# leonardsiegert/PULPo

Measured on AMD Instinct MI355X. Metric: volume-pairs/sec fwd+bwd, 160^3 fp32, higher is better.
Workload: dtype f32

## Files before the change

include/pulpo_hip.h:

```cpp
#ifndef PULPO_HIP_H
#define PULPO_HIP_H

#include <stddef.h>
#include <stdint.h>

#ifdef __cplusplus
extern "C" {
#endif

#define PULPO_ABI_VERSION 8
int pulpo_abi_version(void);
const char* pulpo_last_error(void);

size_t pulpo_conv3d_k3_packed_floats(int K, int N);
int pulpo_conv3d_k3_pack_weight(const float* w , float* wp, int Cin, int Cout, int dgrad, void* stream);
int pulpo_conv3d_k3_stat_tiles(int B, int D, int H, int W);
int pulpo_conv3d_k3_tile_config(int K, int N);
size_t pulpo_conv3d_k3_fwd_scratch_floats(int B, int D, int H, int W, int K, int N);
int pulpo_conv3d_k3_fwd(const float* in, int64_t in_bs, int64_t in_ps, int64_t in_cs, const float* wp, const float* bias, float* out,
                        int64_t out_bs, int64_t out_ps, int64_t out_cs, float* stats, float* scratch , int B,
                        int D, int H, int W, int K, int N, void* stream);
int pulpo_conv3d_k3_fwd_bn_lrelu(const float* in, int64_t in_bs, int64_t in_ps, int64_t in_cs, const float* wp, const float* bias,
                                 const float* coef, float slope, float* out, int64_t out_bs, int64_t out_ps, int64_t out_cs, float* scratch, int B,
                                 int D, int H, int W, int K, int N, void* stream);
int pulpo_conv3d_k3_algo(int B, int D, int H, int W, int K, int N);
size_t pulpo_conv3d_k3_packed_wino2_floats(int K, int N);
int pulpo_conv3d_k3_pack_weight_wino2(const float* w , float* wp, int Cin, int Cout, int dgrad, void* stream);
size_t pulpo_conv3d_k3_fwd_wino2_scratch_floats(int B, int D, int H, int W, int K, int N);
int pulpo_conv3d_k3_fwd_wino2(const float* in, int64_t in_bs, int64_t in_ps, int64_t in_cs, const float* wp, const float* bias, const float* coef,
                              float slope, float* out, int64_t out_bs, int64_t out_ps, int64_t out_cs, float* stats,
                              float* scratch , int B, int D, int H, int W, int K, int N, void* stream);
int pulpo_conv3d_k3_wino2_pipelined(int D, int H, int W, int K, int64_t in_ps);
int pulpo_conv3d_k3_dgrad_wino2_bnred_ok(int B, int D, int H, int W, int K, int N);
int pulpo_conv3d_k3_dgrad_wino2_bnred(const float* in, int64_t in_bs, int64_t in_ps, int64_t in_cs, const float* wp, float* out, int64_t out_bs,
                                      int64_t out_ps, const float* bn_y, int64_t bn_y_bs, int64_t bn_y_ps, const float* bn_coef, float slope,
                                      float* part, int B, int D, int H, int W, int K, int N, void* stream);
typedef struct PulpoPackJob {
    const float* w;
    float* wp;
    int Cin, Cout, dgrad, kind;
} PulpoPackJob;
int pulpo_conv3d_k3_pack_weights_multi(const PulpoPackJob* jobs, int njobs, void* stream);
size_t pulpo_conv3d_k3_wgrad_scratch_floats(int Cin, int Cout);
int pulpo_conv3d_k3_wgrad_algo(int B, int D, int H, int W, int Cin, int Cout, int vec);
int pulpo_conv3d_k3_wgrad(const float* in, int64_t in_bs, int64_t in_ps, int64_t in_cs, const float* dy, int64_t dy_bs, int64_t dy_ps,
                          int64_t dy_cs, float* dw, int accumulate, float* scratch, int B, int D, int H, int W, int Cin,
                          int Cout, void* stream);
typedef struct PulpoGradJob {
    const float* src;
    float* dst;
    int kind, a, b, c;
} PulpoGradJob;
int pulpo_grad_finish_multi(const PulpoGradJob* jobs, int njobs, void* stream);

size_t pulpo_conv3d_k3_packed_bf16_elems(int K, int N);
int pulpo_conv3d_k3_pack_weight_bf16(const float* w , uint16_t* wp, int Cin, int Cout, int dgrad, void* stream);
size_t pulpo_conv3d_k3_fwd_bf16_scratch_floats(int B, int D, int H, int W, int K, int N);
int pulpo_conv3d_k3_fwd_bf16_stat_tiles(int B, int D, int H, int W);
int pulpo_conv3d_k3_fwd_bf16(const float* in, int64_t in_bs, int64_t in_ps, int64_t in_cs, const uint16_t* wp, const float* bias, float* out,
                             int64_t out_bs, int64_t out_ps, int64_t out_cs, float* stats, float* scratch, int B, int D, int H, int W, int K,
                             int N, void* stream);
int pulpo_conv3d_k3_fwd_bn_lrelu_bf16(const float* in, int64_t in_bs, int64_t in_ps, int64_t in_cs, const uint16_t* wp, const float* bias,
                                      const float* coef, float slope, float* out, int64_t out_bs, int64_t out_ps, int64_t out_cs, float* scratch,
                                      int B, int D, int H, int W, int K, int N, void* stream);
int pulpo_conv3d_k3_wgrad_bf16(const float* in, int64_t in_bs, int64_t in_ps, int64_t in_cs, const float* dy, int64_t dy_bs, int64_t dy_ps,
                               int64_t dy_cs, float* dw, int accumulate, float* scratch , int B, int D,
                               int H, int W, int Cin, int Cout, void* stream);

int pulpo_colsum(const float* partials, int nrow, int ncol, float* out, float scale, int accumulate, void* stream);
size_t pulpo_bn_fwd_finalize_scratch_doubles(int ntile, int C);
int pulpo_bn_fwd_finalize(const float* stats, int ntile, int C, double count, const float* gamma, const float* beta, float* running_mean,
                          float* running_var, int64_t* num_batches_tracked , float momentum, float eps, float* coef,
                          double* scratch, void* stream);
int pulpo_bn_eval_coef(const float* gamma, const float* beta, const float* running_mean, const float* running_var, float eps, int C,
                       float* coef, void* stream);
int pulpo_bn_lrelu_apply(const float* y, int64_t yps, float* z, int64_t zps, const float* coef, int64_t npix, int C, float slope, void* stream);
int pulpo_bn_lrelu_apply_pool2_ok(int C, int64_t yps, int64_t zps, int64_t pps);
int pulpo_bn_lrelu_apply_pool2(const float* y, int64_t yps, float* z, int64_t zps, float* pooled, int64_t pps, const float* coef, int B, int D, int H,
                               int W, int C, float slope, void* stream);
int pulpo_bn_bwd_blocks(int64_t npix, int C);
int pulpo_avgpool2_bwd_bnred(const float* gout, int64_t gops, const float* add, int64_t aps, float* gin, int64_t gips, const float* y, int64_t yps,
                             const float* coef, float slope, float* partial, int B, int D, int H, int W, int C, void* stream);
int pulpo_bn_lrelu_bwd_reduce(const float* dz, int64_t dzps, const float* y, int64_t yps, const float* coef, int64_t npix, int C, float slope,
                              float* partial , void* stream);
size_t pulpo_bn_bwd_finalize_scratch_doubles(int nrow, int C);
int pulpo_bn_bwd_finalize(const float* rows, int nrow, int C, const float* coef, double count, int use_means, float* dbeta, float* dgamma,
                          int accumulate, double* totd , double* scratch, void* stream);
int pulpo_bn_lrelu_bwd_apply(const float* dz, int64_t dzps, const float* y, int64_t yps, const float* coef, const double* totd, float* dy,
                             int64_t dyps, int64_t npix, int C, float slope, float* partial2 , void* stream);

int pulpo_heads_fwd(const float* h, int64_t ps, const float* Wt, const float* bias, const float* eps, float* o0, float* o1, float* o2, int nout,
                    int B, int64_t V, int C, void* stream);
int pulpo_heads_bwd_blocks(int B, int64_t V, int C);
int pulpo_heads_bwd(const float* h, int64_t ps, const float* Wt, const float* g0, const float* g1, const float* g2, const float* eps,
                    const float* sigma, float* dh, int64_t dps, float* partial , int nout, int B, int64_t V, int C,
                    void* stream);

int pulpo_avgpool2_fwd(const float* in, int64_t ips, float* out, int64_t ops, int B, int D, int H, int W, int C, void* stream);
int pulpo_avgpool2_bwd(const float* gout, int64_t gops, float* gin, int64_t gips, int B, int D, int H, int W, int C, void* stream);
int pulpo_avgpool2_bwd_add(const float* gout, int64_t gops, const float* add, int64_t aps, float* gin, int64_t gips, int B, int D, int H, int W,
                           int C, void* stream);
int pulpo_resize_trilinear_fwd(const float* in, const float* add, float* out, int64_t nplanes, int Di, int Hi, int Wi, int Do, int Ho, int Wo,
                               float mult, void* stream);
int pulpo_resize_trilinear_bwd(const float* gout, float* gin, int64_t nplanes, int Di, int Hi, int Wi, int Do, int Ho, int Wo, float mult,
                               void* stream);
int pulpo_resize_trilinear_scaled_fwd(const float* in, const float* add, float* out, int64_t nplanes, int Di, int Hi, int Wi, int Do, int Ho,
                                      int Wo, float scale_d, float scale_h, float scale_w, float mult, void* stream);
int pulpo_resize_trilinear_scaled_bwd(const float* gout, float* gin, int64_t nplanes, int Di, int Hi, int Wi, int Do, int Ho, int Wo,
                                      float scale_d, float scale_h, float scale_w, float mult, void* stream);
int pulpo_feedback_up2_fwd(const float* const* srcs , const int* chans , int nsrc, float* out, int64_t ops,
                           int B, int Di, int Hi, int Wi, void* stream);
int pulpo_feedback_up2_bwd(const float* gout, int64_t gops, float* const* gsrcs , const int* chans, int nsrc,
                           int B, int Di, int Hi, int Wi, void* stream);

int pulpo_warp3d_fwd(const float* df, const float* img, float* out, int B, int C, int Dg, int Hg, int Wg, int Di, int Hi, int Wi, void* stream);
int pulpo_warp_mask_fwd(const float* df, const float* mask, float* out, int B, int Dg, int Hg, int Wg, int Di, int Hi, int Wi, void* stream);
int pulpo_warp3d_bwd(const float* df, const float* img, const float* gout, float* gdf, float* gimg, int B, int C, int Dg, int Hg, int Wg, int Di,
                     int Hi, int Wi, void* stream);
int pulpo_vecint_fwd(const float* v, float* work, int B, int D, int H, int W, int nsteps, void* stream);
size_t pulpo_vecint_bwd_tmp_floats(int B, int D, int H, int W, int nsteps);
int pulpo_vecint_bwd(const float* work, const float* gout, float* gin, float* tmp , int B, int D, int H, int W,
                     int nsteps, void* stream);

int pulpo_loss_blocks(int64_t n);
int pulpo_ncc_fwd(const float* I, const float* J, float* S , float* T , float* partial, int B, int D, int H, int W,
                  int win, void* stream);
int pulpo_ncc_bwd(const float* I, const float* J, const float* S, float* T , const float* gscale, float coef, float* gJ, int B, int D,
                  int H, int W, int win, void* stream);
int pulpo_ncc_masked_fwd(const float* I, const float* J, const float* wa, const float* wb , float* S ,
                         float* T , float* partial , int B, int D, int H, int W, int win, void* stream);
int pulpo_ncc_masked_bwd(const float* I, const float* J, const float* S, const float* wa, const float* wb , float* T ,
                         const float* gscale, float coef, float* gJ, int B, int D, int H, int W, int win, void* stream);
int pulpo_masked_finish(const float* partial, int nblk, double scale, int root, double count, float* out , void* stream);
int pulpo_mind_blocks(int B, int D, int H, int W, int d);
int pulpo_mind_descriptor(const float* I, float* out , int B, int D, int H, int W, int d, float eps, void* stream);
int pulpo_mind_fwd(const float* y_true, const float* y_pred, const float* wa , const float* wb , float* partial, int B, int D,
                   int H, int W, int d, float eps, void* stream);
int pulpo_mind_bwd(const float* y_true, const float* y_pred, const float* wa , const float* wb , float* scratch ,
                   const float* gscale, float coef, float* gpred, int B, int D, int H, int W, int d, float eps, void* stream);
int pulpo_mi_blocks(int B, int64_t V);
int64_t pulpo_mi_scratch_floats(int B, int64_t V, int K);
int pulpo_mi_fwd(const float* y_true, const float* y_pred, const float* wa , const float* wb , float* scratch, double* p,
                 double* mi, float* G, float* loss, int B, int64_t V, int K, double gamma, void* stream);
int pulpo_mi_bwd(const float* y_true, const float* y_pred, const float* wa , const float* wb , const float* G,
                 const float* gscale, float coef, float* gpred, int B, int64_t V, int K, void* stream);
int pulpo_kl_fwd(const float* mu, const float* sigma, const float* mu1 , const float* sigma1 , int64_t n,
                 float* partial, void* stream);
int pulpo_kl_bwd(const float* mu, const float* sigma, const float* mu1, const float* sigma1, const float* gscale, float coef, float* gmu,
                 float* gsigma, int64_t n, void* stream);
int pulpo_l2reg_fwd(const float* df, int64_t nplanes, int D, int H, int W, float* partial, void* stream);
int pulpo_l2reg_bwd(const float* df, const float* gscale, float coef, float* gdf, int64_t nplanes, int D, int H, int W, void* stream);
int pulpo_bending_blocks(int64_t nplanes, int D, int H, int W);
int pulpo_bending_fwd(const float* df, int64_t nplanes, int D, int H, int W, float* partial, void* stream);
int pulpo_bending_bwd(const float* df, const float* gscale, float coef, float* gdf, int64_t nplanes, int D, int H, int W, void* stream);
int pulpo_weighted_sum_fwd(const float* terms, const float* weights, int n, float scale, int scaled, float* levels, float* total, void* stream);
int pulpo_weighted_sum_bwd(const float* gtotal, const float* glevels, const float* weights, int n, float scale, float* gterms, void* stream);

int pulpo_metric_blocks(int64_t n);
int pulpo_sqdiff_fwd(const float* a, const float* b, int64_t n, float* partial, void* stream);
int pulpo_sqdiff_bwd(const float* a, const float* b, const float* gscale, float coef, float* ga, int64_t n, void* stream);
int pulpo_sqdiff_masked_fwd(const float* a, const float* b, const float* wa, const float* wb ,
                            float* partial , int B, int C, int64_t V, void* stream);
int pulpo_sqdiff_masked_bwd(const float* a, const float* b, const float* wa, const float* wb , const float* gscale, float coef, float* ga,
                            int B, int C, int64_t V, void* stream);
int pulpo_dice_blocks(int64_t V);
int pulpo_dice_fwd(const float* inp, const float* tgt, int nplanes, int64_t V, float dice_factor, float* partial, double* numden, float* loss,
                   void* stream);
int pulpo_dice_bwd(const float* inp, const float* tgt, const double* numden, const float* gscale, int nplanes, int64_t V, float dice_factor,
                   float* ginp, void* stream);
int pulpo_jacdet_fwd(const float* df, float* out, double* partial , int B, int D, int H, int W, int normalize, void* stream);
int pulpo_jdetstd_finalize(const double* partial, int64_t n, float lamb, double* stat, float* loss, void* stream);
int pulpo_kl_nondiag_fwd(const float* mu, const float* sigma, int64_t nplanes, int D, int H, int W, float prior_lambda, float* partial, float* loss,
                         void* stream);
int pulpo_kl_nondiag_bwd(const float* mu, const float* sigma, const float* gscale, int64_t nplanes, int D, int H, int W, float prior_lambda,
                         float* gmu, float* gsigma, void* stream);
int pulpo_jdetstd_bwd(const float* df, const float* jdet, const double* stat, const float* gscale, float lamb, float* gdf, int B, int D, int H, int W,
                      int normalize, void* stream);

int pulpo_rmse(const float* a, const float* b, int64_t n, float* partial , float* out, void* stream);
int pulpo_dsc(const float* inp, const float* tgt, int nplanes, int64_t V, float* partial , float* out,
              void* stream);
int pulpo_percent_leq0(const float* x, int64_t n, float* partial , float* out, void* stream);
int pulpo_warp_landmarks(const float* lm , const float* df , float* out , int nlm, int nsamp,
                         int nd, int D, int H, int W, int* flag, void* stream);
int pulpo_field_quality_blocks(int B, int D, int H, int W);
size_t pulpo_field_quality_ws_bytes(int B, int D, int H, int W);
int pulpo_field_quality(const float* df, float* out , void* ws, int B, int D, int H, int W, int normalize, void* stream);

size_t pulpo_vecint_pair_scratch_floats(int B, int D, int H, int W, int nsteps);
int pulpo_vecint_pair_fwd(const float* v, float* fwd, float* inv, float* scratch , int B, int D, int H, int W, int nsteps,
                          void* stream);
size_t pulpo_inverse_consistency_ws_bytes(int B, int D, int H, int W);
int pulpo_inverse_consistency(const float* a, const float* b, float* out , void* ws, int B, int D, int H, int W, void* stream);
int pulpo_transport_points(const float* pts , const float* field , float* out , int npts,
                           int nsamp, int nd, int D, int H, int W, int* flag, void* stream);

int pulpo_affine_field(const float* theta, float* out, int B, int D, int H, int W, void* stream);
int pulpo_affine_warp_fwd(const float* theta, const float* img, float* out, int B, int C, int Dg, int Hg, int Wg, int Di, int Hi, int Wi, void* stream);
size_t pulpo_affine_warp_bwd_ws_bytes(int B, int Dg, int Hg, int Wg);
int pulpo_affine_warp_bwd(const float* theta, const float* img, const float* gout, float* gtheta , void* ws, int B, int C, int Dg, int Hg,
                          int Wg, int Di, int Hi, int Wi, void* stream);
int pulpo_affine_compose(const float* theta, const float* df, float* out, int B, int Dg, int Hg, int Wg, int Di, int Hi, int Wi, void* stream);

int pulpo_mc_moments_update(const float* sample, float* mean, float* m2, int64_t n, int k, void* stream);
int pulpo_mc_moments_std(const float* m2, const float* scale , float* out , int B, int C, int64_t V, int k, void* stream);

size_t pulpo_warp_labels_ws_bytes(int B, int C);
int pulpo_warp_labels(const float* df, const void* labels, int ldt, int C, const void* target , float* onehot ,
                      void* amax , float* dice , float* mean , float* m2 ,
                      int k, void* ws, int* flag, int B, int Dg, int Hg, int Wg, int Di, int Hi, int Wi, void* stream);
int pulpo_labels_check(const void* labels, int ldt, int64_t n, int C, int* flag, void* stream);
int pulpo_warp_labels_soft_dice(const float* df, const void* labels, const void* target, int ldt, int C, float* dice, float* mean, void* ws,
                                int* flag, int B, int Dg, int Hg, int Wg, int Di, int Hi, int Wi, int Dt, int Ht, int Wt, void* stream);
int pulpo_labels_from_onehot(const float* seg, void* labels, int ldt, int B, int C, int64_t V, void* stream);
int pulpo_map_ncc_blocks(int64_t n);
int pulpo_map_ncc(const float* a, const float* b, int64_t n, double* partial, double* out, void* stream);
int pulpo_label_dice_fwd(const float* df, const void* labels, const void* target, int ldt, int C, float dice_factor, float* loss, float* dice,
                         float* coef, void* ws, int* flag, int B, int Dg, int Hg, int Wg, int Di, int Hi, int Wi, int Dt, int Ht, int Wt,
                         void* stream);
int pulpo_label_dice_bwd(const float* df, const void* labels, const void* target, int ldt, int C, const float* coef, const float* gup, float* ddf,
                         int B, int Dg, int Hg, int Wg, int Di, int Hi, int Wi, int Dt, int Ht, int Wt, void* stream);
int pulpo_labels_pool2(const void* labels, int ldt, int C, float* out, int B, int D, int H, int W, void* stream);
int pulpo_labels_resize(const void* labels, int ldt, int C, float* out, int B, int Dt, int Ht, int Wt, int Do, int Ho, int Wo, void* stream);

#define PULPO_EDT_INF (1 << 29)
int pulpo_edt_sq(const void* mask, int* out, int B, int D, int H, int W, void* stream);
int64_t pulpo_surface_distances_bins(int D, int H, int W);
size_t pulpo_surface_distances_ws_bytes(int B, int C, int D, int H, int W);
int pulpo_surface_distances(const void* lab_a, const void* lab_b, int ldt, int C, double q, float* out, int* hist , void* ws, int* flag,
                            int B, int D, int H, int W, int nd, void* stream);

int pulpo_augment_apply(const float* theta, const float* phi, int spacing, int Gz, int Gy, int Gx, const float* img, float* img_out, int C,
                        const float* mask, float* mask_out, int Cm, const void* labels, void* labels_out, int ldt, const float* iparams, int iflags,
                        const float* bias, int Lz, int Ly, int Lx, const void* seed, float fill, int fill_label, int B, int D, int H, int W,
                        void* stream);
int pulpo_bspline_field(const float* phi, const float* theta, float* out, int spacing, int Gz, int Gy, int Gx, int B, int D, int H, int W, void* stream);
int pulpo_philox4x32(const void* counters, const void* key, void* out, int64_t n, void* stream);

int pulpo_adam_step(float* p, const float* g, float* m, float* v, int64_t n, float lr, double beta1, double beta2, float eps, int step, float gscale,
                    void* stream);
int pulpo_anchored_adam_step(float* p, const float* g, float* m, float* v, const float* mean, const float* prec, int64_t n, float lr, double beta1,
                             double beta2, float eps, int step, float* partial, void* stream);

size_t pulpo_conv3d_k3_packed_wino3_floats(int K, int N);
int pulpo_conv3d_k3_pack_weight_wino3(const float* w , float* wp, int Cin, int Cout, int dgrad, void* stream);
int pulpo_conv3d_k3_fwd_wino3(const float* in, int64_t in_bs, int64_t in_ps, int64_t in_cs, const float* wp, const float* bias, const float* coef,
                              float slope, float* out, int64_t out_bs, int64_t out_ps, int64_t out_cs, float* stats, int B, int D, int H, int W, int K,
                              int N, void* stream);
int pulpo_conv3d_k3_dgrad_wino3_bnred(const float* in, int64_t in_bs, int64_t in_ps, int64_t in_cs, const float* wp, float* out, int64_t out_bs,
                                      int64_t out_ps, const float* bn_y, int64_t bn_y_bs, int64_t bn_y_ps, const float* bn_coef, float slope, float* part,
                                      int B, int D, int H, int W, int K, int N, void* stream);
int pulpo_conv3d_k3_wino3g_ok(int B, int D, int H, int W, int K, int N);
size_t pulpo_conv3d_k3_fwd_wino3g_scratch_floats(int B, int D, int H, int W, int K, int N);
int pulpo_conv3d_k3_fwd_wino3g(const float* in, int64_t in_bs, int64_t in_ps, int64_t in_cs, const float* wp, const float* bias, const float* coef,
                               float slope, float* out, int64_t out_bs, int64_t out_ps, int64_t out_cs, float* stats, float* scratch, int B, int D,
                               int H, int W, int K, int N, void* stream);

int pulpo_conv3d_k3_fwd_bf16_t(const void* in, int64_t in_bs, int64_t in_ps, int64_t in_cs, const uint16_t* wp, const float* bias, void* out,
                               int64_t out_bs, int64_t out_ps, int64_t out_cs, int dt, float* stats, float* scratch, int B, int D, int H, int W,
                               int K, int N, void* stream);
int pulpo_conv3d_k3_fwd_bn_lrelu_bf16_t(const void* in, int64_t in_bs, int64_t in_ps, int64_t in_cs, const uint16_t* wp, const float* bias,
                                        const float* coef, float slope, void* out, int64_t out_bs, int64_t out_ps, int64_t out_cs, int dt,
                                        float* scratch, int B, int D, int H, int W, int K, int N, void* stream);
int pulpo_conv3d_k3_wgrad_bf16_t(const void* in, int64_t in_bs, int64_t in_ps, int64_t in_cs, const void* dy, int64_t dy_bs, int64_t dy_ps,
                                 int64_t dy_cs, int dt, float* dw, int accumulate, float* scratch, int B, int D, int H, int W, int Cin, int Cout,
                                 void* stream);
int pulpo_conv3d_k3_fwd_bf16_kernel(int B, int D, int H, int W, int K, int N, int dt, int64_t in_ps, int64_t out_ps);
int pulpo_conv3d_k3_wgrad_bf16_kernel(int B, int D, int H, int W, int Cin, int Cout, int dt, int64_t in_ps, int64_t dy_ps);
int pulpo_bn_lrelu_apply_t(const void* y, int y_dt, int64_t yps, void* z, int z_dt, int64_t zps, const float* coef, int64_t npix, int C, float slope,
                           void* stream);
int pulpo_bn_lrelu_apply_pool2_t(const void* y, int y_dt, int64_t yps, void* z , int z_dt, int64_t zps,
                                 void* pooled , int64_t pps,
                                 const float* coef, int B, int D, int H, int W, int C, float slope, void* stream);
int pulpo_bn_lrelu_bwd_reduce_t(const void* dz, int dz_dt, int64_t dzps, const void* y, int y_dt, int64_t yps, const float* coef, int64_t npix, int C,
                                float slope, float* partial, void* stream);
int pulpo_bn_lrelu_bwd_apply_t(const void* dz, int dz_dt, int64_t dzps, const void* y, int y_dt, int64_t yps, const float* coef, const double* totd,
                               void* dy , int64_t dyps, int64_t npix, int C, float slope, float* partial2, void* stream);
int pulpo_avgpool2_bwd_bnred_t(const void* gout, int64_t gops, const void* add, int64_t aps, void* gin, int64_t gips, int g_dt ,
                               const void* y, int y_dt, int64_t yps, const float* coef, float slope, float* partial, int B, int D, int H, int W,
                               int C, void* stream);
int pulpo_heads_fwd_t(const void* h, int h_dt, int64_t ps, const float* Wt, const float* bias, const float* eps, float* o0, float* o1, float* o2,
                      int nout, int B, int64_t V, int C, void* stream);
int pulpo_heads_bwd_t(const void* h, int h_dt, int64_t ps, const float* Wt, const float* g0, const float* g1, const float* g2, const float* eps,
                      const float* sigma, void* dh , int64_t dps, float* partial, int nout, int B, int64_t V, int C, void* stream);
int pulpo_avgpool2_fwd_t(const void* in, int64_t ips, void* out, int64_t ops, int dt, int B, int D, int H, int W, int C, void* stream);
int pulpo_avgpool2_bwd_t(const void* gout, int64_t gops, const void* add , int64_t aps, void* gin, int64_t gips, int dt, int B, int D,
                         int H, int W, int C, void* stream);
int pulpo_feedback_up2_fwd_t(const float* const* srcs , const int* chans , int nsrc, void* out,
                             int dt, int64_t ops, int B, int Di, int Hi, int Wi, void* stream);
int pulpo_feedback_up2_bwd_t(const void* gout, int dt, int64_t gops, float* const* gsrcs , const int* chans,
                             int nsrc, int B, int Di, int Hi, int Wi, void* stream);

int pulpo_conv3d_k3_wgrad_bn_rows(int B, int D, int H, int W, int Cout);
int pulpo_conv3d_k3_wgrad_bn(const float* in, int64_t in_bs, int64_t in_ps, int64_t in_cs, const void* dz, int dz_dt, int64_t dz_bs, int64_t dz_ps,
                             const float* y, int64_t y_bs, int64_t y_ps, const float* coef, const double* totd, float slope, float* dw,
                             int accumulate, float* scratch, float* part2, int B, int D, int H, int W, int Cin, int Cout, void* stream);

int pulpo_bn_lrelu_bwd_apply_pooled_t(const void* gout, int64_t gops, const void* add , int64_t aps, int g_dt, const void* y, int y_dt,
                                      int64_t yps, const float* coef, const double* totd, void* dy , int64_t dyps, float slope,
                                      float* partial2, int B, int D, int H, int W, int C, void* stream);

int pulpo_bn_lrelu_apply_kb(const float* y, int64_t yps, float* z, int64_t zps, int64_t zkb, const float* coef, int64_t npix, int C, float slope, void* stream);
int pulpo_bn_lrelu_bwd_apply_kb_t(const void* dz, int dz_dt, int64_t dzps, int64_t dzkb, const float* y, int64_t yps, const float* coef, const double* totd,
                                  float* dy, int64_t dyps, int64_t dykb, int64_t npix, int C, float slope, float* partial2, void* stream);
int pulpo_conv3d_k3_wgrad_bn_kb(const float* in, int64_t in_bs, int64_t in_ps, int64_t in_cs, const float* dz, int64_t dz_bs, int64_t dz_ps, int64_t dz_kb,
                                const float* y, int64_t y_bs, int64_t y_ps, const float* coef, const double* totd, float slope, float* dw, int accumulate,
                                float* scratch, float* part2, int B, int D, int H, int W, int Cin, int Cout, void* stream);
int pulpo_bn_lrelu_bwd_apply_pooled_kb_t(const void* gout, int64_t gops, const void* add , int64_t aps, int g_dt, const float* y, int64_t yps,
                                         const float* coef, const double* totd, float* dy, int64_t dyps, int64_t dykb, float slope, float* partial2,
                                         int B, int D, int H, int W, int C, void* stream);
int pulpo_conv3d_k3_fwd_wino3_kb(const float* in, int64_t in_bs, int64_t in_ps, int64_t in_kb, const float* wp, const float* bias, const float* coef,
                                 float slope, float* out, int64_t out_bs, int64_t out_ps, int64_t out_kb, float* stats, int B, int D, int H, int W, int K,
                                 int N, void* stream);
int pulpo_conv3d_k3_dgrad_wino3_bnred_kb(const float* in, int64_t in_bs, int64_t in_ps, int64_t in_kb, const float* wp, float* out, int64_t out_bs,
                                         int64_t out_ps, int64_t out_kb, const float* bn_y, int64_t bn_y_bs, int64_t bn_y_ps, const float* bn_coef, float slope,
                                         float* part, int B, int D, int H, int W, int K, int N, void* stream);
int pulpo_conv3d_k3_wgrad_kb(const float* in, int64_t in_bs, int64_t in_ps, int64_t in_kb, const float* dy, int64_t dy_bs, int64_t dy_ps, int64_t dy_kb,
                             float* dw, int accumulate, float* scratch, float* slabs , int nslab, int B, int D, int H, int W, int Cin, int Cout,
                             void* stream);

int pulpo_conv3d_k3_wgrad_det_slabs(int Cin, int Cout);
int pulpo_conv3d_k3_wgrad_det(const float* in, int64_t in_bs, int64_t in_ps, int64_t in_cs, const float* dy, int64_t dy_bs, int64_t dy_ps,
                              int64_t dy_cs, float* dw, int accumulate, float* scratch, float* slabs, int nslab, int B, int D, int H, int W,
                              int Cin, int Cout, void* stream);
int pulpo_conv3d_k3_wgrad_bf16_det_t(const void* in, int64_t in_bs, int64_t in_ps, int64_t in_cs, const void* dy, int64_t dy_bs, int64_t dy_ps,
                                     int64_t dy_cs, int dt, float* dw, int accumulate, float* scratch, float* slabs, int nslab, int B, int D,
                                     int H, int W, int Cin, int Cout, void* stream);
int pulpo_resize_trilinear_scaled_bwd_det(const float* gout, float* gin, int64_t nplanes, int Di, int Hi, int Wi, int Do, int Ho, int Wo,
                                          float scale_d, float scale_h, float scale_w, float mult, void* stream);
size_t pulpo_warp3d_bwd_det_ws_bytes(int B, int C, int Di, int Hi, int Wi);
int pulpo_warp3d_bwd_det(const float* df, const float* img, const float* gout, float* gdf , float* gimg ,
                         void* ws , int B, int C, int Dg, int Hg, int Wg, int Di, int Hi, int Wi, void* stream);
size_t pulpo_vecint_bwd_det_ws_bytes(int B, int D, int H, int W, int nsteps);
int pulpo_vecint_bwd_det(const float* work, const float* gout, float* gin, void* ws , int B, int D, int H, int W,
                         int nsteps, void* stream);

int pulpo_conv3d_k3_wgrad_grid(int B, int D, int H, int W, int Cin, int Cout, int max_workgroups);
int pulpo_conv3d_k3_wgrad_wg(const float* in, int64_t in_bs, int64_t in_ps, int64_t in_cs, const float* dy, int64_t dy_bs, int64_t dy_ps,
                             int64_t dy_cs, float* dw, int accumulate, float* scratch, int B, int D, int H, int W, int Cin, int Cout, void* stream,
                             int max_workgroups);
int pulpo_conv3d_k3_wgrad_det_wg(const float* in, int64_t in_bs, int64_t in_ps, int64_t in_cs, const float* dy, int64_t dy_bs, int64_t dy_ps,
                                 int64_t dy_cs, float* dw, int accumulate, float* scratch, float* slabs, int nslab, int B, int D, int H, int W,
                                 int Cin, int Cout, void* stream, int max_workgroups);
int pulpo_conv3d_k3_wgrad_kb_wg(const float* in, int64_t in_bs, int64_t in_ps, int64_t in_kb, const float* dy, int64_t dy_bs, int64_t dy_ps, int64_t dy_kb,
                                float* dw, int accumulate, float* scratch, float* slabs , int nslab, int B, int D, int H, int W, int Cin, int Cout,
                                void* stream, int max_workgroups);

int pulpo_heads_fwd_bn_t(const float* y, int64_t ps, const float* coef, float slope, const float* Wt, const float* bias, const float* eps ,
                         float* o0, float* o1, float* o2, int nout, int B, int64_t V, int C, void* stream);
int pulpo_heads_bwd_bn_t(const float* y, int64_t ps, const float* coef, float slope, const float* Wt, const float* g0, const float* g1, const float* g2,
                         const float* eps, const float* sigma, float* partial , float* bnpart , int nout, int B,
                         int64_t V, int C, void* stream);
int pulpo_bn_lrelu_bwd_apply_heads_t(const float* y, int64_t yps, const float* coef, const double* totd, float slope, const float* Wt, const float* g0,
                                     const float* g1, const float* g2, const float* eps, const float* sigma, float* dy, int64_t dyps, float* partial2,
                                     int nout, int B, int64_t V, int C, void* stream);
int pulpo_bn_lrelu_bwd_apply_heads_kb_t(const float* y, int64_t yps, const float* coef, const double* totd, float slope, const float* Wt, const float* g0,
                                        const float* g1, const float* g2, const float* eps, const float* sigma, float* dy, int64_t dyps, int64_t dykb,
                                        float* partial2, int nout, int B, int64_t V, int C, void* stream);

#ifdef __cplusplus
}
#endif
#endif
```

pulpo_amd/csrc/conv3d_wgrad_w2.hip:

```cpp
#include "conv_shared.h"
#include <type_traits>

namespace {

using namespace pulpo_conv;
using f32x2 = __attribute__((ext_vector_type(2))) float;

constexpr int W2G_VROW = 44, W2G_EROW = 36;
constexpr int W2G_VSLOT = 32 * W2G_VROW, W2G_ESLOT = 32 * W2G_EROW;
constexpr int W2G_VX = 4 * 4 * W2G_VSLOT;
constexpr int W2G_EX = 4 * 2 * W2G_ESLOT;
constexpr size_t W2G_LDS = (size_t)(W2G_VX + W2G_EX) * sizeof(float);

struct Wgrad2Args {
    const float* in;
    long in_bs, in_ps;
    const float* go;
    long go_bs, go_ps;
    float* dwp;
    int B, D, H, W, Cin, Cout, NPad;
    int nty, ntx, ncit, ncot, nsplit;
    long split_stride;
    long in_kb;
    long go_kb;
};

template <int DUMMY>
__global__ __launch_bounds__(256, 1) void conv3d_k3_wgrad_w2(Wgrad2Args a) {
    extern __shared__ __attribute__((aligned(16))) float smem[];
    float* VX = smem;
    float* EX = smem + W2G_VX;

    const int tid = threadIdx.x, lane = tid & 63, wave = __builtin_amdgcn_readfirstlane(tid >> 6);
    const int i = lane & 31, kk = lane >> 5;
    const int py = wave;
    const int lid = pulpo::xcd_remap(blockIdx.x, gridDim.x);
    const int npair = a.ncit * a.ncot;
    const int pair = lid % npair, split = lid / npair;
    const int cit = pair / a.ncot, cot = pair - cit * a.ncot;
    const int ci0 = cit * 32, co0 = cot * 32;

    const int ta = py == 0 ? 0 : py == 2 ? 2 : 1;
    const int tb = py == 2 ? 1 : py == 3 ? 3 : 2;
    const float sa = py == 1 ? 1.f : -1.f;
    const float c0 = py == 3 ? 0.f : 1.f;
    const float c1 = py == 0 ? 0.f : py == 1 ? 1.f : -1.f;

    const int ncol = a.B * a.nty * a.ntx;
    const long nstep = (long)ncol * a.D;
    const long p_begin = nstep * split / a.nsplit, p_end = nstep * (split + 1) / a.nsplit;

    const int it_q = tid & 7, it_xb = (tid >> 3) & 3, it_y = tid >> 5;
    const bool xb_item = tid < 64;
    const bool x_cok = ci0 + 4 * it_q < a.Cin, e_cok = co0 + 4 * it_q < a.Cout;
    float* const xa_dst = VX + (4 * it_q) * W2G_VROW + it_y * 4 + it_xb;
    float* const xb_dst = xa_dst + 8 * 4;
    float* const e_dst = EX + (4 * it_q) * W2G_EROW + it_y * 4 + it_xb;

    unsigned xa_ok = 0, xb_ok = 0, e_ok = 0;
    const float* xa_src = a.in;
    const float* e_src = a.go;
    auto set_column = [&](int col) {
        int t = col;
        const int tx_ = t % a.ntx; t /= a.ntx;
        const int ty_ = t % a.nty;
        const int cb = t / a.nty;
        const int y0 = ty_ * 8, x0 = tx_ * 8;
        const int gy = y0 - 1 + it_y;
        xa_ok = 0; xb_ok = 0; e_ok = 0;
#pragma unroll
        for (int t4 = 0; t4 < 4; ++t4) {
            const bool xin = (unsigned)(x0 - 1 + 2 * it_xb + t4) < (unsigned)a.W;
            if (x_cok && xin && (unsigned)gy < (unsigned)a.H) xa_ok |= 1u << t4;
            if (xb_item && x_cok && xin && (unsigned)(gy + 8) < (unsigned)a.H) xb_ok |= 1u << t4;
        }
        xa_src = a.in + (long)cb * a.in_bs + ((long)gy * a.W + (x0 - 1 + 2 * it_xb)) * a.in_ps + ci0 + 4 * it_q;
        const int ey = y0 + it_y;
#pragma unroll
        for (int t2 = 0; t2 < 2; ++t2)
            if (e_cok && ey < a.H && x0 + 2 * it_xb + t2 < a.W) e_ok |= 1u << t2;
        e_src = a.go + (long)cb * a.go_bs + ((long)ey * a.W + (x0 + 2 * it_xb)) * a.go_ps + co0 + 4 * it_q;
    };
    const long x_plane = (long)a.H * a.W * a.in_ps, e_plane = (long)a.H * a.W * a.go_ps;
    const long x_rows8 = 8L * a.W * a.in_ps;

    float4 xra[4], xrb[4], er[2];
    auto issue_x = [&](int zp) {
        const bool zok = (unsigned)zp < (unsigned)a.D;
        const float* src = xa_src + (long)zp * x_plane;
#pragma unroll
        for (int t4 = 0; t4 < 4; ++t4) {
            xra[t4] = make_float4(0.f, 0.f, 0.f, 0.f);
            if (zok && ((xa_ok >> t4) & 1u)) xra[t4] = *reinterpret_cast<const float4*>(src + (long)t4 * a.in_ps);
            xrb[t4] = make_float4(0.f, 0.f, 0.f, 0.f);
            if (zok && ((xb_ok >> t4) & 1u)) xrb[t4] = *reinterpret_cast<const float4*>(src + x_rows8 + (long)t4 * a.in_ps);
        }
    };
    auto issue_e = [&](int zp) {
        const bool zok = (unsigned)zp < (unsigned)a.D;
#pragma unroll
        for (int t2 = 0; t2 < 2; ++t2) {
            er[t2] = make_float4(0.f, 0.f, 0.f, 0.f);
            if (zok && ((e_ok >> t2) & 1u)) er[t2] = *reinterpret_cast<const float4*>(e_src + (long)zp * e_plane + (long)t2 * a.go_ps);
        }
    };
    auto write_x = [&](const float4 (&d)[4], float* dst, int px, int slot) {
        const float4 d0 = d[0], d1 = d[1], d2 = d[2], d3 = d[3];
        float4 v;
        if (px == 0) v = make_float4(d0.x - d2.x, d0.y - d2.y, d0.z - d2.z, d0.w - d2.w);
        else if (px == 1) v = make_float4(d1.x + d2.x, d1.y + d2.y, d1.z + d2.z, d1.w + d2.w);
        else if (px == 2) v = make_float4(d2.x - d1.x, d2.y - d1.y, d2.z - d1.z, d2.w - d1.w);
        else v = make_float4(d1.x - d3.x, d1.y - d3.y, d1.z - d3.z, d1.w - d3.w);
        float* o = dst + (px * 4 + slot) * W2G_VSLOT;
        o[0] = v.x; o[W2G_VROW] = v.y; o[2 * W2G_VROW] = v.z; o[3 * W2G_VROW] = v.w;
    };
    auto write_e = [&](int px, int slot) {
        const float4 d0 = er[0], d1 = er[1];
        float4 v;
        if (px == 0) v = d0;
        else if (px == 1) v = make_float4(d0.x + d1.x, d0.y + d1.y, d0.z + d1.z, d0.w + d1.w);
        else if (px == 2) v = make_float4(d0.x - d1.x, d0.y - d1.y, d0.z - d1.z, d0.w - d1.w);
        else v = make_float4(-d1.x, -d1.y, -d1.z, -d1.w);
        float* o = e_dst + (px * 2 + slot) * W2G_ESLOT;
        o[0] = v.x; o[W2G_EROW] = v.y; o[2 * W2G_EROW] = v.z; o[3 * W2G_EROW] = v.w;
    };
    auto stage_part = [&](int k, int xslot, int eslot) {
        write_x(xra, xa_dst, k, xslot);
        write_e(k, eslot);
        if (xb_item) write_x(xrb, xb_dst, k, xslot);
    };
    auto touch_raw = [&]() {
#pragma unroll
        for (int t4 = 0; t4 < 4; ++t4) {
            asm volatile("" : : "v"(xra[t4].x), "v"(xra[t4].y), "v"(xra[t4].z), "v"(xra[t4].w));
            asm volatile("" : : "v"(xrb[t4].x), "v"(xrb[t4].y), "v"(xrb[t4].z), "v"(xrb[t4].w));
        }
#pragma unroll
        for (int t2 = 0; t2 < 2; ++t2) asm volatile("" : : "v"(er[t2].x), "v"(er[t2].y), "v"(er[t2].z), "v"(er[t2].w));
    };

    f32x16 acc[4][3];
#pragma unroll
    for (int p = 0; p < 4; ++p)
#pragma unroll
        for (int dz = 0; dz < 3; ++dz)
#pragma unroll
            for (int r = 0; r < 16; ++r) acc[p][dz][r] = 0.f;

    const float* va = VX + i * W2G_VROW + (2 * kk + ta) * 4;
    const float* vb = VX + i * W2G_VROW + (2 * kk + tb) * 4;
    const float* ea = EX + i * W2G_EROW + (2 * kk) * 4;

    long p = p_begin;
    while (p < p_end) {
        const int pc = (int)(p / a.D);
        const int zs = (int)(p - (long)pc * a.D);
        const int ze = (int)min((long)a.D, (long)zs + (p_end - p));
        set_column(pc);
        issue_x(zs - 1);
        er[0] = make_float4(0.f, 0.f, 0.f, 0.f); er[1] = make_float4(0.f, 0.f, 0.f, 0.f);
#pragma unroll 1
        for (int j = zs - 3; j < zs; ++j) {
            __syncthreads();
            touch_raw();
#pragma unroll
            for (int k = 0; k < 4; ++k) stage_part(k, (j + 3) & 3, (j & 1) ^ 1);
            issue_x(j + 3);
            issue_e(j + 2);
        }
#pragma unroll 1
        for (int j = zs; j < ze; ++j) {
            __syncthreads();
            const int xs_slot = (j + 3) & 3, es = j & 1;
            float4 av[2][3], bv[2][3], e0[2], e1[2];
            auto fetch = [&](int gi, int set) {
                const int g = gi >> 2, px = gi & 3;
                const float* eb = ea + (px * 2 + es) * W2G_ESLOT + g * 16;
                e0[set] = *reinterpret_cast<const float4*>(eb);
                e1[set] = *reinterpret_cast<const float4*>(eb + 4);
#pragma unroll
                for (int dz = 0; dz < 3; ++dz) {
                    const int off = (px * 4 + ((j + dz) & 3)) * W2G_VSLOT + g * 16;
                    av[set][dz] = *reinterpret_cast<const float4*>(va + off);
                    bv[set][dz] = *reinterpret_cast<const float4*>(vb + off);
                }
            };
            fetch(0, 0);
#pragma unroll
            for (int gi = 0; gi < 8; ++gi) {
                const int set = gi & 1, px = gi & 3;
                if (gi + 1 < 8) fetch(gi + 1, set ^ 1);
                __builtin_amdgcn_sched_barrier(0);
                const float4 f0 = e0[set], f1 = e1[set];
                const float ev[4] = {fmaf(c1, f1.x, c0 * f0.x), fmaf(c1, f1.y, c0 * f0.y), fmaf(c1, f1.z, c0 * f0.z), fmaf(c1, f1.w, c0 * f0.w)};
#pragma unroll
                for (int dz = 0; dz < 3; ++dz) {
                    const float4 pa_ = av[set][dz], pb_ = bv[set][dz];
                    const float v4[4] = {fmaf(sa, pb_.x, pa_.x), fmaf(sa, pb_.y, pa_.y), fmaf(sa, pb_.z, pa_.z), fmaf(sa, pb_.w, pa_.w)};
#pragma unroll
                    for (int s_ = 0; s_ < 4; ++s_) acc[px][dz] = __builtin_amdgcn_mfma_f32_32x32x2f32(v4[s_], ev[s_], acc[px][dz], 0, 0, 0);
                    if (dz == 0 && gi < 4) {
                        __builtin_amdgcn_sched_barrier(0);
                        if (gi == 0) touch_raw();
                        stage_part(gi, xs_slot, es ^ 1);
                        if (gi == 3) {
                            issue_x(j + 3);
                            issue_e(j + 2);
                        }
                        __builtin_amdgcn_sched_barrier(0);
                    }
                }
                __builtin_amdgcn_sched_barrier(0);
            }
        }
        p += ze - zs;
        __syncthreads();
    }

    __syncthreads();
    float* X = smem;
    const int Cc = min(32, a.Cin - ci0);
#pragma unroll 1
    for (int dz = 0; dz < 3; ++dz) {
#pragma unroll
        for (int r = 0; r < 16; ++r) {
            const float m0 = dz == 0 ? acc[0][0][r] : dz == 1 ? acc[0][1][r] : acc[0][2][r];
            const float m1 = dz == 0 ? acc[1][0][r] : dz == 1 ? acc[1][1][r] : acc[1][2][r];
            const float m2 = dz == 0 ? acc[2][0][r] : dz == 1 ? acc[2][1][r] : acc[2][2][r];
            const float m3 = dz == 0 ? acc[3][0][r] : dz == 1 ? acc[3][1][r] : acc[3][2][r];
            const float hs = 0.5f * (m1 + m2);
            X[((py * 3 + 0) * 16 + r) * 64 + lane] = m0 + hs;
            X[((py * 3 + 1) * 16 + r) * 64 + lane] = 0.5f * (m1 - m2);
            X[((py * 3 + 2) * 16 + r) * 64 + lane] = hs + m3;
        }
        __syncthreads();
        for (int e = tid; e < 3 * 16 * 64; e += 256) {
            const int l = e & 63, r = (e >> 6) & 15, kx = e >> 10;
            float s4[4];
#pragma unroll
            for (int q = 0; q < 4; ++q) s4[q] = X[((q * 3 + kx) * 16 + r) * 64 + l];
            const int ci = (r & 3) + 8 * (r >> 2) + 4 * (l >> 5), co = co0 + (l & 31);
            if (ci < Cc && co < a.Cout) {
                const float hs = 0.5f * (s4[1] + s4[2]);
                float* d = a.dwp + (long)split * a.split_stride + ((long)((dz * 3 + 0) * 3 + kx) * a.Cin + ci0 + ci) * a.NPad + co;
                const long kystride = 3L * a.Cin * a.NPad;
                atomicAdd(d, s4[0] + hs);
                atomicAdd(d + kystride, 0.5f * (s4[1] - s4[2]));
                atomicAdd(d + 2 * kystride, hs + s4[3]);
            }
        }
        __syncthreads();
    }
}

template <int DUMMY>
__global__ __launch_bounds__(512, 2) void conv3d_k3_wgrad_w2x(Wgrad2Args a) {
    extern __shared__ __attribute__((aligned(16))) float smem[];
    float* VX = smem;
    float* EX = smem + W2G_VX;

    const int tid = threadIdx.x, lane = tid & 63, wave = __builtin_amdgcn_readfirstlane(tid >> 6);
    const int i = lane & 31, kk = lane >> 5;
    const int py = wave & 3, pxh = wave >> 2;
    const int lid = pulpo::xcd_remap(blockIdx.x, gridDim.x);
    const int npair = a.ncit * a.ncot;
    const int pair = lid % npair, split = lid / npair;
    const int cit = pair / a.ncot, cot = pair - cit * a.ncot;
    const int ci0 = cit * 32, co0 = cot * 32;

    const int ta = py == 0 ? 0 : py == 2 ? 2 : 1;
    const int tb = py == 2 ? 1 : py == 3 ? 3 : 2;
    const float sa = py == 1 ? 1.f : -1.f;
    const float c0 = py == 3 ? 0.f : 1.f;
    const float c1 = py == 0 ? 0.f : py == 1 ? 1.f : -1.f;

    const int ncol = a.B * a.nty * a.ntx;
    const long nstep = (long)ncol * a.D;
    const long p_begin = nstep * split / a.nsplit, p_end = nstep * (split + 1) / a.nsplit;

    const bool x_item = tid < 320;
    const int x_q = tid & 7, x_xb = (tid >> 3) & 3, x_hy = tid >> 5;
    const bool e_item = tid >= 256;
    const int e_t = tid - 256;
    const int e_q = e_t & 7, e_xb = (e_t >> 3) & 3, e_y = (e_t >> 5) & 7;
    const bool x_cok = ci0 + 4 * x_q < a.Cin, e_cok = co0 + 4 * e_q < a.Cout;
    float* const x_dst = VX + (4 * x_q) * W2G_VROW + x_hy * 4 + x_xb;
    float* const e_dst = EX + (4 * e_q) * W2G_EROW + e_y * 4 + e_xb;

    constexpr unsigned OOB = 0x80000000u;
    const int x_bytes = (int)((long)a.D * a.H * a.W * a.in_ps * 4), e_bytes = (int)((long)a.D * a.H * a.W * a.go_ps * 4);
    int cb = 0, y0 = 0, x0 = 0;
    unsigned x_off[4], e_off[2];
    __amdgpu_buffer_rsrc_t x_rs = __builtin_amdgcn_make_buffer_rsrc(const_cast<float*>(a.in), 0, x_bytes, 0x00020000);
    __amdgpu_buffer_rsrc_t e_rs = __builtin_amdgcn_make_buffer_rsrc(const_cast<float*>(a.go), 0, e_bytes, 0x00020000);
    auto set_column = [&](int col) {
        int t = col;
        const int tx_ = t % a.ntx; t /= a.ntx;
        const int ty_ = t % a.nty;
        cb = t / a.nty;
        y0 = ty_ * 8; x0 = tx_ * 8;
        x_rs = __builtin_amdgcn_make_buffer_rsrc(const_cast<float*>(a.in + (long)cb * a.in_bs), 0, x_bytes, 0x00020000);
        e_rs = __builtin_amdgcn_make_buffer_rsrc(const_cast<float*>(a.go + (long)cb * a.go_bs), 0, e_bytes, 0x00020000);
        const int gy = y0 - 1 + x_hy;
        const bool xrow = x_item && x_cok && (unsigned)gy < (unsigned)a.H;
#pragma unroll
        for (int t4 = 0; t4 < 4; ++t4) {
            const int gx = x0 - 1 + 2 * x_xb + t4;
            x_off[t4] = (xrow && (unsigned)gx < (unsigned)a.W) ? (unsigned)((gy * a.W + gx) * (int)a.in_ps + ci0 + 4 * x_q) * 4u : OOB;
        }
        const int ey = y0 + e_y;
        const bool erow = e_item && e_cok && ey < a.H;
#pragma unroll
        for (int t2 = 0; t2 < 2; ++t2) {
            const int gx = x0 + 2 * e_xb + t2;
            e_off[t2] = (erow && gx < a.W) ? (unsigned)((ey * a.W + gx) * (int)a.go_ps + co0 + 4 * e_q) * 4u : OOB;
        }
    };
    const unsigned x_plane = (unsigned)((long)a.H * a.W * a.in_ps * 4), e_plane = (unsigned)((long)a.H * a.W * a.go_ps * 4);

    float4 xr[4], er[2];
    auto issue_x = [&](int zp) {
        const unsigned zmask = (unsigned)zp < (unsigned)a.D ? 0u : OOB;
        const unsigned zo = zmask ? 0u : (unsigned)zp * x_plane;
#pragma unroll
        for (int t4 = 0; t4 < 4; ++t4)
            xr[t4] = __builtin_bit_cast(float4, __builtin_amdgcn_raw_buffer_load_b128(x_rs, (int)(x_off[t4] | zmask), (int)zo, 0));
    };
    auto issue_e = [&](int zp) {
        const unsigned zmask = (unsigned)zp < (unsigned)a.D ? 0u : OOB;
        const unsigned zo = zmask ? 0u : (unsigned)zp * e_plane;
#pragma unroll
        for (int t2 = 0; t2 < 2; ++t2)
            er[t2] = __builtin_bit_cast(float4, __builtin_amdgcn_raw_buffer_load_b128(e_rs, (int)(e_off[t2] | zmask), (int)zo, 0));
    };
    auto write_x = [&](int px, int slot) {
        if (x_item) {
            const float4 pa_ = px == 0 ? xr[0] : px == 2 ? xr[2] : xr[1], pb_ = px == 0 ? xr[2] : px == 1 ? xr[2] : px == 2 ? xr[1] : xr[3];
            const f32x2 sg = px == 1 ? f32x2{1.f, 1.f} : f32x2{-1.f, -1.f};
            const f32x2 lo = f32x2{pa_.x, pa_.y} + sg * f32x2{pb_.x, pb_.y}, hi = f32x2{pa_.z, pa_.w} + sg * f32x2{pb_.z, pb_.w};
            const float4 v = make_float4(lo.x, lo.y, hi.x, hi.y);
            float* o = x_dst + (px * 4 + slot) * W2G_VSLOT;
            o[0] = v.x; o[W2G_VROW] = v.y; o[2 * W2G_VROW] = v.z; o[3 * W2G_VROW] = v.w;
        }
    };
    auto write_e = [&](int px, int slot) {
        if (e_item) {
            const float4 d0 = er[0], d1 = er[1];
            float4 v;
            if (px == 0) v = d0;
            else if (px == 3) v = make_float4(-d1.x, -d1.y, -d1.z, -d1.w);
            else {
                const f32x2 sg = px == 1 ? f32x2{1.f, 1.f} : f32x2{-1.f, -1.f};
                const f32x2 lo = f32x2{d0.x, d0.y} + sg * f32x2{d1.x, d1.y}, hi = f32x2{d0.z, d0.w} + sg * f32x2{d1.z, d1.w};
                v = make_float4(lo.x, lo.y, hi.x, hi.y);
            }
            float* o = e_dst + (px * 2 + slot) * W2G_ESLOT;
            o[0] = v.x; o[W2G_EROW] = v.y; o[2 * W2G_EROW] = v.z; o[3 * W2G_EROW] = v.w;
        }
    };
    auto touch_raw = [&]() {
#pragma unroll
        for (int t4 = 0; t4 < 4; ++t4) asm volatile("" : : "v"(xr[t4].x), "v"(xr[t4].y), "v"(xr[t4].z), "v"(xr[t4].w));
#pragma unroll
        for (int t2 = 0; t2 < 2; ++t2) asm volatile("" : : "v"(er[t2].x), "v"(er[t2].y), "v"(er[t2].z), "v"(er[t2].w));
    };

    f32x16 acc[2][3];
#pragma unroll
    for (int p = 0; p < 2; ++p)
#pragma unroll
        for (int dz = 0; dz < 3; ++dz)
#pragma unroll
            for (int r = 0; r < 16; ++r) acc[p][dz][r] = 0.f;

    const float* va = VX + i * W2G_VROW + (2 * kk + ta) * 4;
    const float* vb = VX + i * W2G_VROW + (2 * kk + tb) * 4;
    const float* ea = EX + i * W2G_EROW + (2 * kk) * 4;

    long p = p_begin;
    while (p < p_end) {
        const int pc = (int)(p / a.D);
        const int zs = (int)(p - (long)pc * a.D);
        const int ze = (int)min((long)a.D, (long)zs + (p_end - p));
        set_column(pc);
        issue_x(zs - 1);
        er[0] = make_float4(0.f, 0.f, 0.f, 0.f); er[1] = make_float4(0.f, 0.f, 0.f, 0.f);
#pragma unroll 1
        for (int j = zs - 3; j < zs; ++j) {
            __syncthreads();
            touch_raw();
#pragma unroll
            for (int gi = 0; gi < 4; ++gi) {
                write_x(gi, (j + 3) & 3);
                write_e(gi, (j & 1) ^ 1);
            }
            issue_x(j + 3);
            issue_e(j + 2);
        }
#pragma unroll 1
        for (int j = zs; j < ze; ++j) {
            __syncthreads();
            const int xs_slot = (j + 3) & 3, es = j & 1;
            float4 av[3], bv[3], e0, e1;
#pragma unroll
            for (int gi = 0; gi < 4; ++gi) {
                const int g = gi >> 1, px = 2 * pxh + (gi & 1), pl = gi & 1;
                const float* eb = ea + (px * 2 + es) * W2G_ESLOT + g * 16;
                e0 = *reinterpret_cast<const float4*>(eb);
                e1 = *reinterpret_cast<const float4*>(eb + 4);
#pragma unroll
                for (int dz = 0; dz < 3; ++dz) {
                    const int off = (px * 4 + ((j + dz) & 3)) * W2G_VSLOT + g * 16;
                    av[dz] = *reinterpret_cast<const float4*>(va + off);
                    bv[dz] = *reinterpret_cast<const float4*>(vb + off);
                }
                __builtin_amdgcn_sched_barrier(0);
                const f32x2 c0v = {c0, c0}, c1v = {c1, c1}, sav = {sa, sa};
                const f32x2 e01 = __builtin_elementwise_fma(c1v, f32x2{e1.x, e1.y}, c0v * f32x2{e0.x, e0.y});
                const f32x2 e23 = __builtin_elementwise_fma(c1v, f32x2{e1.z, e1.w}, c0v * f32x2{e0.z, e0.w});
                const float ev[4] = {e01.x, e01.y, e23.x, e23.y};
                float vv[3][4];
#pragma unroll
                for (int dz = 0; dz < 3; ++dz) {
                    const float4 pa_ = av[dz], pb_ = bv[dz];
                    const f32x2 v01 = __builtin_elementwise_fma(sav, f32x2{pb_.x, pb_.y}, f32x2{pa_.x, pa_.y});
                    const f32x2 v23 = __builtin_elementwise_fma(sav, f32x2{pb_.z, pb_.w}, f32x2{pa_.z, pa_.w});
                    vv[dz][0] = v01.x; vv[dz][1] = v01.y; vv[dz][2] = v23.x; vv[dz][3] = v23.y;
                }
                __builtin_amdgcn_sched_barrier(0);
#pragma unroll
                for (int dz = 0; dz < 3; ++dz) {
#pragma unroll
                    for (int s_ = 0; s_ < 4; ++s_) acc[pl][dz] = __builtin_amdgcn_mfma_f32_32x32x2f32(vv[dz][s_], ev[s_], acc[pl][dz], 0, 0, 0);
                    if (dz == 0 && gi < 2) {
                        __builtin_amdgcn_sched_barrier(0);
                        if (gi == 0) touch_raw();
                        write_x(2 * gi, xs_slot);
                        write_x(2 * gi + 1, xs_slot);
                        write_e(2 * gi, es ^ 1);
                        write_e(2 * gi + 1, es ^ 1);
                        if (gi == 1) {
                            issue_x(j + 3);
                            issue_e(j + 2);
                        }
                        __builtin_amdgcn_sched_barrier(0);
                    }
                }
                __builtin_amdgcn_sched_barrier(0);
            }
        }
        p += ze - zs;
        __syncthreads();
    }

    __syncthreads();
    float* X = smem;
    const int Cc = min(32, a.Cin - ci0);
#pragma unroll 1
    for (int dz = 0; dz < 3; ++dz) {
#pragma unroll
        for (int r = 0; r < 16; ++r) {
            const float m0 = dz == 0 ? acc[0][0][r] : dz == 1 ? acc[0][1][r] : acc[0][2][r];
            const float m1 = dz == 0 ? acc[1][0][r] : dz == 1 ? acc[1][1][r] : acc[1][2][r];
            float t0, t1, t2;
            if (pxh == 0) { t0 = m0 + 0.5f * m1; t1 = 0.5f * m1; t2 = 0.5f * m1; }
            else { t0 = 0.5f * m0; t1 = -0.5f * m0; t2 = 0.5f * m0 + m1; }
            X[((wave * 3 + 0) * 16 + r) * 64 + lane] = t0;
            X[((wave * 3 + 1) * 16 + r) * 64 + lane] = t1;
            X[((wave * 3 + 2) * 16 + r) * 64 + lane] = t2;
        }
        __syncthreads();
        for (int e = tid; e < 3 * 16 * 64; e += 512) {
            const int l = e & 63, r = (e >> 6) & 15, kx = e >> 10;
            float s[4];
#pragma unroll
            for (int q = 0; q < 4; ++q)
                s[q] = X[((q * 3 + kx) * 16 + r) * 64 + l] + X[(((q + 4) * 3 + kx) * 16 + r) * 64 + l];
            const int ci = (r & 3) + 8 * (r >> 2) + 4 * (l >> 5), co = co0 + (l & 31);
            if (ci < Cc && co < a.Cout) {
                const float hs = 0.5f * (s[1] + s[2]);
                float* d = a.dwp + (long)split * a.split_stride + ((long)((dz * 3 + 0) * 3 + kx) * a.Cin + ci0 + ci) * a.NPad + co;
                const long kystride = 3L * a.Cin * a.NPad;
                atomicAdd(d, s[0] + hs);
                atomicAdd(d + kystride, 0.5f * (s[1] - s[2]));
                atomicAdd(d + 2 * kystride, hs + s[3]);
            }
        }
        __syncthreads();
    }
}

constexpr int W3G_EX = 4 * 4 * W2G_ESLOT;
constexpr size_t W3G_LDS = (size_t)(W2G_VX + W3G_EX) * sizeof(float);


template <int SG>
__device__ __forceinline__ void wgrad_w3x_body(const Wgrad2Args& a) {
    extern __shared__ __attribute__((aligned(16))) float smem[];
    float* VX = smem;
    float* EX = smem + W2G_VX;

    const int tid = threadIdx.x, lane = tid & 63, wave = __builtin_amdgcn_readfirstlane(tid >> 6);
    const int i = lane & 31, kk = lane >> 5;
    const int py = wave & 3, pxh = wave >> 2;
    const int lid = pulpo::xcd_remap(blockIdx.x, gridDim.x);
    const int npair = a.ncit * a.ncot;
    const int pair = lid % npair, split = lid / npair;
    const int cit = pair / a.ncot, cot = pair - cit * a.ncot;
    const int ci0 = cit * 32, co0 = cot * 32;

    const int ta = py == 0 ? 0 : py == 2 ? 2 : 1;
    const int tb = py == 2 ? 1 : py == 3 ? 3 : 2;
    const float sa = py == 1 ? 1.f : -1.f;
    const int ea_ = py == 3 ? 1 : 0, eb_ = py == 0 ? 0 : 1;
    const float se = py == 0 ? 0.f : py == 1 ? 1.f : py == 2 ? -1.f : -2.f;

    const int ncol = a.B * a.nty * a.ntx;
    const int DP = a.D >> 1;
    const long nstep = (long)ncol * DP;
    const long p_begin = nstep * split / a.nsplit, p_end = nstep * (split + 1) / a.nsplit;

    const bool x_item = tid < 320;
    const int x_q = tid & 7, x_xb = (tid >> 3) & 3, x_hy = tid >> 5;
    const bool e_item = tid >= 256;
    const int e_t = tid - 256;
    const int e_q = e_t & 7, e_xb = (e_t >> 3) & 3, e_y = (e_t >> 5) & 7;
    const bool x_cok = ci0 + 4 * x_q < a.Cin, e_cok = co0 + 4 * e_q < a.Cout;
    float* const x_dst = VX + x_q * W2G_VROW + x_hy * 4 + x_xb;
    float* const e_dst = EX + e_q * W2G_EROW + e_y * 4 + e_xb;
    const int x_d4 = ((x_q ^ 4) - x_q) * W2G_VROW, e_d4 = ((e_q ^ 4) - e_q) * W2G_EROW;

    constexpr unsigned OOB = 0x80000000u;
    const int x_bytes = (int)((((long)(a.Cin + 7) / 8 - 1) * (a.in_kb == 8 ? 0 : a.in_kb) + (long)a.D * a.H * a.W * a.in_ps) * 4);
    const int e_bytes = (int)((((long)(a.Cout + 7) / 8 - 1) * (a.go_kb == 8 ? 0 : a.go_kb) + (long)a.D * a.H * a.W * a.go_ps) * 4);
    int cb = 0, y0 = 0, x0 = 0;
    unsigned x_off[4], e_off[2];
    __amdgpu_buffer_rsrc_t x_rs = __builtin_amdgcn_make_buffer_rsrc(const_cast<float*>(a.in), 0, x_bytes, 0x00020000);
    __amdgpu_buffer_rsrc_t e_rs = __builtin_amdgcn_make_buffer_rsrc(const_cast<float*>(a.go), 0, e_bytes, 0x00020000);
    auto set_column = [&](int col) {
        int t = col;
        const int tx_ = t % a.ntx; t /= a.ntx;
        const int ty_ = t % a.nty;
        cb = t / a.nty;
        y0 = ty_ * 8; x0 = tx_ * 8;
        x_rs = __builtin_amdgcn_make_buffer_rsrc(const_cast<float*>(a.in + (long)cb * a.in_bs), 0, x_bytes, 0x00020000);
        e_rs = __builtin_amdgcn_make_buffer_rsrc(const_cast<float*>(a.go + (long)cb * a.go_bs), 0, e_bytes, 0x00020000);
        const int gy = y0 - 1 + x_hy;
        const bool xrow = x_item && x_cok && (unsigned)gy < (unsigned)a.H;
#pragma unroll
        for (int t4 = 0; t4 < 4; ++t4) {
            const int gx = x0 - 1 + 2 * x_xb + t4;
            x_off[t4] = (xrow && (unsigned)gx < (unsigned)a.W) ? (unsigned)((long)((ci0 + 4 * x_q) >> 3) * a.in_kb + (gy * a.W + gx) * (int)a.in_ps + ((4 * x_q) & 7)) * 4u : OOB;
        }
        const int ey = y0 + e_y;
        const bool erow = e_item && e_cok && ey < a.H;
#pragma unroll
        for (int t2 = 0; t2 < 2; ++t2) {
            const int gx = x0 + 2 * e_xb + t2;
            e_off[t2] = (erow && gx < a.W) ? (unsigned)((long)((co0 + 4 * e_q) >> 3) * a.go_kb + (ey * a.W + gx) * (int)a.go_ps + ((4 * e_q) & 7)) * 4u : OOB;
        }
    };
    const unsigned x_plane = (unsigned)((long)a.H * a.W * a.in_ps * 4), e_plane = (unsigned)((long)a.H * a.W * a.go_ps * 4);

    float4 xr[4], er[2];
    auto issue_x = [&](int zp) {
        const unsigned zmask = (unsigned)zp < (unsigned)a.D ? 0u : OOB;
        const unsigned zo = zmask ? 0u : (unsigned)zp * x_plane;
#pragma unroll
        for (int t4 = 0; t4 < 4; ++t4)
            xr[t4] = __builtin_bit_cast(float4, __builtin_amdgcn_raw_buffer_load_b128(x_rs, (int)(x_off[t4] | zmask), (int)zo, 0));
    };
    auto issue_e = [&](int zp) {
        const unsigned zmask = (unsigned)zp < (unsigned)a.D ? 0u : OOB;
        const unsigned zo = zmask ? 0u : (unsigned)zp * e_plane;
#pragma unroll
        for (int t2 = 0; t2 < 2; ++t2)
            er[t2] = __builtin_bit_cast(float4, __builtin_amdgcn_raw_buffer_load_b128(e_rs, (int)(e_off[t2] | zmask), (int)zo, 0));
    };
    auto write_x = [&](int px, int slot) {
        if (x_item) {
            const float4 pa_ = px == 0 ? xr[0] : px == 2 ? xr[2] : xr[1], pb_ = px == 0 ? xr[2] : px == 1 ? xr[2] : px == 2 ? xr[1] : xr[3];
            const f32x2 sg = px == 1 ? f32x2{1.f, 1.f} : f32x2{-1.f, -1.f};
            const f32x2 lo = f32x2{pa_.x, pa_.y} + sg * f32x2{pb_.x, pb_.y}, hi = f32x2{pa_.z, pa_.w} + sg * f32x2{pb_.z, pb_.w};
            const float4 v = make_float4(lo.x, lo.y, hi.x, hi.y);
            float* o = x_dst + (px * 4 + slot) * W2G_VSLOT;
            o[0] = v.x; o[8 * W2G_VROW] = v.y; o[16 * W2G_VROW + x_d4] = v.z; o[24 * W2G_VROW + x_d4] = v.w;
        }
    };
    auto write_e = [&](int px, int slot) {
        if (e_item) {
            const float4 d0 = er[0], d1 = er[1];
            float4 v;
            if (px == 0) v = d0;
            else if (px == 3) v = make_float4(-d1.x, -d1.y, -d1.z, -d1.w);
            else {
                const f32x2 sg = px == 1 ? f32x2{1.f, 1.f} : f32x2{-1.f, -1.f};
                const f32x2 lo = f32x2{d0.x, d0.y} + sg * f32x2{d1.x, d1.y}, hi = f32x2{d0.z, d0.w} + sg * f32x2{d1.z, d1.w};
                v = make_float4(lo.x, lo.y, hi.x, hi.y);
            }
            float* o = e_dst + (px * 4 + slot) * W2G_ESLOT;
            o[0] = v.x; o[8 * W2G_EROW] = v.y; o[16 * W2G_EROW + e_d4] = v.z; o[24 * W2G_EROW + e_d4] = v.w;
        }
    };
    auto touch_raw = [&]() {
#pragma unroll
        for (int t4 = 0; t4 < 4; ++t4) asm volatile("" : : "v"(xr[t4].x), "v"(xr[t4].y), "v"(xr[t4].z), "v"(xr[t4].w));
#pragma unroll
        for (int t2 = 0; t2 < 2; ++t2) asm volatile("" : : "v"(er[t2].x), "v"(er[t2].y), "v"(er[t2].z), "v"(er[t2].w));
    };

    f32x16 acc[2][4];
#pragma unroll
    for (int p = 0; p < 2; ++p)
#pragma unroll
        for (int pz = 0; pz < 4; ++pz)
#pragma unroll
            for (int r = 0; r < 16; ++r) acc[p][pz][r] = 0.f;

    const int irow = 8 * (i & 3) + ((i >> 2) ^ (4 * ((i >> 1) & 1)));
    const float* va = VX + irow * W2G_VROW + (2 * kk + ta) * 4;
    const float* vb = VX + irow * W2G_VROW + (2 * kk + tb) * 4;
    const float* ea = EX + irow * W2G_EROW + (2 * kk) * 4;

    long p = p_begin;
    while (p < p_end) {
        const int pc = (int)(p / DP);
        const int Js = (int)(p - (long)pc * DP);
        const int Je = (int)min((long)DP, (long)Js + (p_end - p));
        set_column(pc);
        const int hs = 2 * Js;
        issue_x(hs - 1);
        issue_e(hs);
#pragma unroll 1
        for (int h = hs - 3; h < hs; ++h) {
            __syncthreads();
            touch_raw();
#pragma unroll
            for (int gi = 0; gi < 4; ++gi) {
                write_x(gi, (h + 3) & 3);
                write_e(gi, (h + 2) & 3);
            }
            issue_x(h + 3);
            issue_e(h + 3 < hs ? hs : h + 3);
        }
        auto half_step = [&](int h, auto hm_tag) {
            constexpr int HM = decltype(hm_tag)::value;
            constexpr bool HB = (HM & 1) != 0;
            __syncthreads();
            constexpr int xs_slot = (HM + 3) & 3, ew_slot = (HM + 2) & 3;
            constexpr int d0s = (HB ? HM - 1 : HM) & 3, d1s = (HB ? HM : HM + 1) & 3;
            float4 av[3], bv[3], e0[2], e1[2];
#pragma unroll
            for (int gi = 0; gi < 4; ++gi) {
                const int g = gi >> 1, px = 2 * pxh + (gi & 1), pl = gi & 1;
                const float* eb0 = ea + (px * 4 + d0s) * W2G_ESLOT + g * 16;
                const float* eb1 = ea + (px * 4 + d1s) * W2G_ESLOT + g * 16;
                e0[0] = *reinterpret_cast<const float4*>(eb0 + 4 * ea_); e1[0] = *reinterpret_cast<const float4*>(eb0 + 4 * eb_);
                e0[1] = *reinterpret_cast<const float4*>(eb1 + 4 * ea_); e1[1] = *reinterpret_cast<const float4*>(eb1 + 4 * eb_);
#pragma unroll
                for (int dz = 0; dz < 3; ++dz) {
                    const int off = (px * 4 + ((HM + dz) & 3)) * W2G_VSLOT + g * 16;
                    av[dz] = *reinterpret_cast<const float4*>(va + off);
                    bv[dz] = *reinterpret_cast<const float4*>(vb + off);
                }
                __builtin_amdgcn_sched_barrier(0);
                const f32x2 sev = {se, se}, sav = {sa, sa};
                f32x2 P[3][2], E[2][2];
#pragma unroll
                for (int dz = 0; dz < 3; ++dz) {
                    const float4 pa_ = av[dz], pb_ = bv[dz];
                    P[dz][0] = __builtin_elementwise_fma(sav, f32x2{pb_.x, pb_.y}, f32x2{pa_.x, pa_.y});
                    P[dz][1] = __builtin_elementwise_fma(sav, f32x2{pb_.z, pb_.w}, f32x2{pa_.z, pa_.w});
                }
#pragma unroll
                for (int d = 0; d < 2; ++d) {
                    E[d][0] = __builtin_elementwise_fma(sev, f32x2{e1[d].x, e1[d].y}, f32x2{e0[d].x, e0[d].y});
                    E[d][1] = __builtin_elementwise_fma(sev, f32x2{e1[d].z, e1[d].w}, f32x2{e0[d].z, e0[d].w});
                }
                f32x2 VA[2], VB[2], EA[2], EB[2];
#pragma unroll
                for (int q = 0; q < 2; ++q) {
                    if (!HB) { VA[q] = P[0][q] - P[2][q]; VB[q] = P[1][q] + P[2][q]; EA[q] = E[0][q]; EB[q] = E[0][q] + E[1][q]; }
                    else { VA[q] = P[1][q] - P[0][q]; VB[q] = P[2][q] - P[0][q]; EA[q] = E[0][q] - E[1][q]; EB[q] = E[1][q]; }
                }
                const float va4[4] = {VA[0].x, VA[0].y, VA[1].x, VA[1].y}, vb4[4] = {VB[0].x, VB[0].y, VB[1].x, VB[1].y};
                const float ea4[4] = {EA[0].x, EA[0].y, EA[1].x, EA[1].y}, eb4[4] = {EB[0].x, EB[0].y, EB[1].x, EB[1].y};
                __builtin_amdgcn_sched_barrier(0);
                constexpr int PZA = HB ? 2 : 0, PZB = HB ? 3 : 1;
#pragma unroll
                for (int s_ = 0; s_ < 4; ++s_) {
                    acc[pl][PZA] = __builtin_amdgcn_mfma_f32_32x32x2f32(va4[s_], ea4[s_], acc[pl][PZA], 0, 0, 0);
                    acc[pl][PZB] = __builtin_amdgcn_mfma_f32_32x32x2f32(vb4[s_], eb4[s_], acc[pl][PZB], 0, 0, 0);
                    if (s_ == 0 && gi >= SG && gi < SG + 2) {
                        __builtin_amdgcn_sched_barrier(0);
                        if (gi == SG) touch_raw();
                        write_x(2 * (gi - SG), xs_slot);
                        write_x(2 * (gi - SG) + 1, xs_slot);
                        write_e(2 * (gi - SG), ew_slot);
                        write_e(2 * (gi - SG) + 1, ew_slot);
                        if (gi == SG + 1) {
                            issue_x(h + 3);
                            issue_e(h + 3);
                        }
                        __builtin_amdgcn_sched_barrier(0);
                    }
                }
                __builtin_amdgcn_sched_barrier(0);
            }
        };
        {
            using H0 = std::integral_constant<int, 0>; using H1 = std::integral_constant<int, 1>;
            using H2 = std::integral_constant<int, 2>; using H3 = std::integral_constant<int, 3>;
            int J = Js;
            if (J < Je && (J & 1)) { half_step(2 * J, H2{}); half_step(2 * J + 1, H3{}); ++J; }
#pragma unroll 1
            for (; J + 1 < Je; J += 2) {
                half_step(2 * J, H0{}); half_step(2 * J + 1, H1{});
                half_step(2 * J + 2, H2{}); half_step(2 * J + 3, H3{});
            }
            if (J < Je) { half_step(2 * J, H0{}); half_step(2 * J + 1, H1{}); }
        }
        p += Je - Js;
        __syncthreads();
    }

    __syncthreads();
    float* X = smem;
    const int Cc = min(32, a.Cin - ci0);
#pragma unroll 1
    for (int dz = 0; dz < 3; ++dz) {
#pragma unroll
        for (int r = 0; r < 16; ++r) {
            const float h0 = 0.5f * (acc[0][1][r] + acc[0][2][r]), h1 = 0.5f * (acc[1][1][r] + acc[1][2][r]);
            const float m0 = dz == 0 ? acc[0][0][r] + h0 : dz == 1 ? 0.5f * (acc[0][1][r] - acc[0][2][r]) : h0 + acc[0][3][r];
            const float m1 = dz == 0 ? acc[1][0][r] + h1 : dz == 1 ? 0.5f * (acc[1][1][r] - acc[1][2][r]) : h1 + acc[1][3][r];
            float t0, t1, t2;
            if (pxh == 0) { t0 = m0 + 0.5f * m1; t1 = 0.5f * m1; t2 = 0.5f * m1; }
            else { t0 = 0.5f * m0; t1 = -0.5f * m0; t2 = 0.5f * m0 + m1; }
            X[((wave * 3 + 0) * 16 + r) * 64 + lane] = t0;
            X[((wave * 3 + 1) * 16 + r) * 64 + lane] = t1;
            X[((wave * 3 + 2) * 16 + r) * 64 + lane] = t2;
        }
        __syncthreads();
        for (int e = tid; e < 3 * 16 * 64; e += 512) {
            const int l = e & 63, r = (e >> 6) & 15, kx = e >> 10;
            float s[4];
#pragma unroll
            for (int q = 0; q < 4; ++q)
                s[q] = X[((q * 3 + kx) * 16 + r) * 64 + l] + X[(((q + 4) * 3 + kx) * 16 + r) * 64 + l];
            const int ci = (r & 3) + 8 * (r >> 2) + 4 * (l >> 5), co = co0 + (l & 31);
            if (ci < Cc && co < a.Cout) {
                const float hs = 0.5f * (s[1] + s[2]);
                float* d = a.dwp + (long)split * a.split_stride + ((long)((dz * 3 + 0) * 3 + kx) * a.Cin + ci0 + ci) * a.NPad + co;
                const long kystride = 3L * a.Cin * a.NPad;
                atomicAdd(d, s[0] + hs);
                atomicAdd(d + kystride, 0.5f * (s[1] - s[2]));
                atomicAdd(d + 2 * kystride, hs + s[3]);
            }
        }
        __syncthreads();
    }
}

template <int DUMMY>
__global__ __launch_bounds__(512, 2) void conv3d_k3_wgrad_w3x(Wgrad2Args a) {
    if (__builtin_amdgcn_readfirstlane(threadIdx.x >> 8) != 0) wgrad_w3x_body<2>(a);
    else wgrad_w3x_body<0>(a);
}

}

namespace pulpo_conv {

bool wgrad_w3_depth_ok(int D) { return D % 2 == 0 && D >= 4; }

int wgrad_w2_splits(int npair, long nstep, int max_workgroups) {
    if (max_workgroups <= 0) return (int)std::min<long>(std::max(1, 256 / npair), nstep);
    int nsplit = (int)std::min<long>(std::max(1, max_workgroups / npair), nstep);
    int m = 8;
    for (int g = npair; g % 2 == 0 && m > 1; g /= 2) m /= 2;
    if (nsplit >= m) nsplit -= nsplit % m;
    return nsplit;
}

int launch_wgrad_w2(const float* in, long in_bs, long in_ps, const float* go, long go_bs, long go_ps, float* scratch, int B, int D, int H, int W,
                    int Cin, int Cout, hipStream_t st, float* slabs, int nslab, int* used_slabs, long go_kb, long in_kb, int max_workgroups) {
    Wgrad2Args a;
    a.split_stride = 0;
    a.go_kb = go_kb; a.in_kb = in_kb;
    auto use_slabs = [&](int nsplit_) -> int {
        if (!slabs) return 0;
        const size_t base = (size_t)27 * Cin * npad(Cout);
        a.dwp = slabs; a.split_stride = (long)base;
        if (used_slabs) *used_slabs = nsplit_;
        hipError_t e = hipMemsetAsync(slabs, 0, (size_t)nsplit_ * base * sizeof(float), st);
        return e == hipSuccess ? 0 : pulpo::fail((int)e, "wgrad slab memset: %s", hipGetErrorString(e));
    };
    a.in = in; a.in_bs = in_bs; a.in_ps = in_ps;
    a.go = go; a.go_bs = go_bs; a.go_ps = go_ps;
    a.dwp = scratch;
    a.B = B; a.D = D; a.H = H; a.W = W; a.Cin = Cin; a.Cout = Cout; a.NPad = npad(Cout);
    a.nty = pulpo::cdiv(H, 8); a.ntx = pulpo::cdiv(W, 8);
    a.ncit = pulpo::cdiv(Cin, 32); a.ncot = pulpo::cdiv(Cout, 32);
    const int npair = a.ncit * a.ncot;
    const long nstep = (long)B * a.nty * a.ntx * D;
    int nsplit = wgrad_w2_splits(npair, nstep, max_workgroups);
    if (slabs) nsplit = std::min(nsplit, nslab);
    a.nsplit = nsplit;
    static bool attr = false;
    if (!attr) {
        hipError_t e = hipFuncSetAttribute(reinterpret_cast<const void*>(&conv3d_k3_wgrad_w2<0>), hipFuncAttributeMaxDynamicSharedMemorySize, (int)W2G_LDS);
        if (e != hipSuccess) return pulpo::fail((int)e, "hipFuncSetAttribute(wgrad w2): %s", hipGetErrorString(e));
        attr = true;
    }
    const bool small32 = (((long)(Cin + 7) / 8 - 1) * (in_kb == 8 ? 0 : in_kb) + (long)D * H * W * in_ps) * 4 < (1L << 31) &&
                         (((long)(Cout + 7) / 8 - 1) * (go_kb == 8 ? 0 : go_kb) + (long)D * H * W * go_ps) * 4 < (1L << 31);
    if ((go_kb != 8 || in_kb != 8) && !(wgrad_w3_depth_ok(D) && small32))
        return pulpo::fail(1, "conv3d_k3_wgrad: channel-blocked operands are read by the F(2x2x2,3x3x3) kernel only (even depth, operands below 2 GiB)");
    if (wgrad_w3_depth_ok(D) && small32) {
        static bool attr3 = false;
        if (!attr3) {
            hipError_t e = hipFuncSetAttribute(reinterpret_cast<const void*>(&conv3d_k3_wgrad_w3x<0>), hipFuncAttributeMaxDynamicSharedMemorySize, (int)W3G_LDS);
            if (e != hipSuccess) return pulpo::fail((int)e, "hipFuncSetAttribute(wgrad w3x): %s", hipGetErrorString(e));
            attr3 = true;
        }
        const long nstep3 = (long)B * a.nty * a.ntx * (D / 2);
        a.nsplit = wgrad_w2_splits(npair, nstep3, max_workgroups);
        if (slabs) a.nsplit = std::min(a.nsplit, nslab);
        if (int rc = use_slabs(a.nsplit)) return rc;
        hipLaunchKernelGGL((conv3d_k3_wgrad_w3x<0>), dim3(npair * a.nsplit), dim3(512), W3G_LDS, st, a);
        return pulpo::check_launch("conv3d_k3_wgrad_w3x");
    }
    const bool small = (long)D * H * W * in_ps * 4 < (1L << 31) && (long)D * H * W * go_ps * 4 < (1L << 31);
    if (small) {
        static bool attr8 = false;
        if (!attr8) {
            hipError_t e = hipFuncSetAttribute(reinterpret_cast<const void*>(&conv3d_k3_wgrad_w2x<0>), hipFuncAttributeMaxDynamicSharedMemorySize, (int)W2G_LDS);
            if (e != hipSuccess) return pulpo::fail((int)e, "hipFuncSetAttribute(wgrad w2x): %s", hipGetErrorString(e));
            attr8 = true;
        }
        if (int rc = use_slabs(nsplit)) return rc;
        hipLaunchKernelGGL((conv3d_k3_wgrad_w2x<0>), dim3(npair * nsplit), dim3(512), W2G_LDS, st, a);
        return pulpo::check_launch("conv3d_k3_wgrad_w2x");
    }
    if (int rc = use_slabs(nsplit)) return rc;
    hipLaunchKernelGGL((conv3d_k3_wgrad_w2<0>), dim3(npair * nsplit), dim3(256), W2G_LDS, st, a);
    return pulpo::check_launch("conv3d_k3_wgrad_w2");
}

}
```

pulpo_amd/csrc/conv3d_wino3.hip:

```cpp
#include "conv_shared.h"
#include "conv_epilogue.h"
#include "wino3_pack.h"

namespace {

using namespace pulpo_conv;
using f32x2 = __attribute__((ext_vector_type(2))) float;

constexpr int Q_CH = 8, Q_NT = 32;
constexpr int Q_PL = HY * 4;
constexpr int Q_PLROWS = 4 * Q_PL + 2;
constexpr int Q_QROWS = 6 * Q_PLROWS;
constexpr int Q_IMG = 2 * Q_QROWS * 4;
static_assert((2 * Q_PLROWS) % 16 == 4 && (Q_QROWS * 4) % 32 == 16, "bank layout");
constexpr int Q_NITEM = 6 * HY * 4 * 2;
constexpr int Q_TAB = 3 * 512;
constexpr int Q_R = 8 * 2 * 16 * 64;
constexpr int Q_RED = 8 * 2 * Q_NT;
constexpr int Q_PART = 8 * 64 * 8;
constexpr size_t Q_LDS = (size_t)(2 * Q_IMG + Q_TAB + Q_R + Q_RED + Q_PART) * sizeof(float);
static_assert(Q_LDS <= 160 * 1024, "one workgroup per CU");


template <bool BNR, int SP>
__device__ __forceinline__ void wino3_body(const ConvArgs& a) {
    constexpr int CH = Q_CH, NT = Q_NT;
    extern __shared__ __attribute__((aligned(16))) float smem[];
    float* const tab = smem + 2 * Q_IMG;
    float* const R = tab + Q_TAB;
    float* const red = R + Q_R;
    float* const part = red + Q_RED;

    const int tid = threadIdx.x, lane = tid & 63, wave = __builtin_amdgcn_readfirstlane(tid >> 6);
    const int i = lane & 31, kk = lane >> 5;
    const int py = wave & 3, pzh = wave >> 2;
    const int nchunk = a.Cin / CH;
    const int nwork = a.B * a.ntz * a.nty * a.ntx * a.ncot;
    const int nwg = gridDim.x;
    const unsigned ps_bytes = (unsigned)a.in_ps * 4u;
    const unsigned kb_bytes = (unsigned)a.in_kb * 4u;

    unsigned roff;
    int lofs;
    {
        const int q = tid & 1, rb = tid >> 1;
        const int xb = rb & 3, hrow = rb >> 2;
        const int hz = hrow / HY, hy = hrow - hz * HY;
        roff = ((unsigned)((hz * a.H + hy) * a.W + 2 * xb) * (unsigned)a.in_ps + 4u * q) * 4u;
        lofs = (q * Q_QROWS + hz * Q_PLROWS + hy * 4 + xb) * 4;
    }
    const bool item = tid < Q_NITEM;
    auto tab_a = [](int p) { return p == 0 ? 0 : p == 2 ? 2 : 1; };
    auto tab_b = [](int p) { return p == 2 ? 1 : p == 3 ? 3 : 2; };
    auto tab_s = [](int p) { return p == 1 ? 1.f : -1.f; };
    const int ta = tab_a(py), tb = tab_b(py);
    const float sa = tab_s(py);
    const int zu = (pzh == 0 ? 0 : 2) * Q_PLROWS * 4, zv = (pzh == 0 ? 1 : 3) * Q_PLROWS * 4, zw = (pzh == 0 ? 2 : 1) * Q_PLROWS * 4;
    const float bw = pzh == 0 ? 1.f : -1.f;
    const int lrow = (i >> 4) * 2 * Q_PLROWS + ((i >> 2) & 3) * 8 + (i & 3);
    const int pa_off = (kk * Q_QROWS + lrow + ta * 4) * 4;
    const int pb_off = (kk * Q_QROWS + lrow + tb * 4) * 4;

    constexpr unsigned OOB = 0x80000000u;
    const __amdgpu_buffer_rsrc_t w_rsrc = __builtin_amdgcn_make_buffer_rsrc(const_cast<float*>(a.wp), 0, -1, 0x00020000);
    const int in_bytes = (int)((((long)a.Cin / CH - 1) * (a.in_kb == CH ? 0 : a.in_kb) + (long)a.D * a.H * a.W * a.in_ps) * 4);
    struct Tile {
        int tile_lin, b, z0, y0, x0, co0;
        unsigned wbase;
    };
    auto describe = [&](int work) {
        Tile t;
        const int cot = work % a.ncot;
        int q = work / a.ncot;
        int tx_, ty_, tz_;
        if (a.tile_order == 1) {
            const int nt = a.ntx * a.nty * a.ntz;
            t.b = q / nt;
            q -= t.b * nt;
            const int blk = q >> 6, w = q & 63;
            const int nbx = a.ntx >> 2, nby = a.nty >> 2;
            const int bx = blk % nbx, by = (blk / nbx) % nby, bz = blk / (nbx * nby);
            tx_ = bx * 4 + (w & 3); ty_ = by * 4 + ((w >> 2) & 3); tz_ = bz * 4 + (w >> 4);
        } else {
            tx_ = q % a.ntx; q /= a.ntx;
            ty_ = q % a.nty; q /= a.nty;
            tz_ = q % a.ntz;
            t.b = q / a.ntz;
        }
        t.tile_lin = ((t.b * a.ntz + tz_) * a.nty + ty_) * a.ntx + tx_;
        t.z0 = tz_ * 4; t.y0 = ty_ * TY; t.x0 = tx_ * TX;
        t.co0 = cot * NT;
        t.wbase = (unsigned)(((2 * pzh) * 16 + py * 4) * a.NPad + t.co0) * (CH * 4u);
        return t;
    };
    unsigned hoff[4];
    auto halo_offsets = [&](const Tile& t) {
        const unsigned origin = (unsigned)(((t.z0 - 1) * a.H + (t.y0 - 1)) * a.W + (t.x0 - 1)) * ps_bytes;
        const int rb = tid >> 1;
        const int xb = rb & 3, hrow = rb >> 2;
        const int hz = hrow / HY, hy = hrow - hz * HY;
        const bool rowok = item && (unsigned)(t.z0 - 1 + hz) < (unsigned)a.D && (unsigned)(t.y0 - 1 + hy) < (unsigned)a.H;
#pragma unroll
        for (int tt = 0; tt < 4; ++tt)
            hoff[tt] = (rowok && (unsigned)(t.x0 - 1 + 2 * xb + tt) < (unsigned)a.W) ? origin + roff + tt * ps_bytes : OOB;
    };
    auto in_rsrc = [&](int b) {
        return __builtin_amdgcn_make_buffer_rsrc(const_cast<float*>(a.in + (long)b * a.in_bs), 0, in_bytes, 0x00020000);
    };
    float4 raw[4];
    auto load_raw = [&](const __amdgpu_buffer_rsrc_t& rs, unsigned c0_bytes, int tt) {
        raw[tt] = __builtin_bit_cast(float4, __builtin_amdgcn_raw_buffer_load_b128(rs, (int)hoff[tt], (int)c0_bytes, 0));
    };
    auto store_item = [&](float* img) {
        if (item) {
            float* o = img + lofs;
            const float4 d0 = raw[0], d1 = raw[1], d2 = raw[2], d3 = raw[3];
            *reinterpret_cast<float4*>(o) = make_float4(d0.x - d2.x, d0.y - d2.y, d0.z - d2.z, d0.w - d2.w);
            *reinterpret_cast<float4*>(o + Q_PL * 4) = make_float4(d1.x + d2.x, d1.y + d2.y, d1.z + d2.z, d1.w + d2.w);
            *reinterpret_cast<float4*>(o + 2 * Q_PL * 4) = make_float4(d2.x - d1.x, d2.y - d1.y, d2.z - d1.z, d2.w - d1.w);
            *reinterpret_cast<float4*>(o + 3 * Q_PL * 4) = make_float4(d1.x - d3.x, d1.y - d3.y, d1.z - d3.z, d1.w - d3.w);
        }
    };
    const unsigned w_chunk_stride = 64u * CH * a.NPad * 4u;
    const unsigned w_pt_stride = (unsigned)CH * a.NPad * 4u;
    const int wl_off = (i * CH + 4 * kk) * 4;
    auto load_w = [&](unsigned wofs, int s) {
        return __builtin_bit_cast(float4, __builtin_amdgcn_raw_buffer_load_b128(w_rsrc, wl_off, (int)(wofs + ((s >> 2) * 16 + (s & 3)) * w_pt_stride), 0));
    };

    const int ctab = a.ncot * NT;
    for (int c = tid; c < ctab; c += 512) {
        const bool in = c < a.Cout;
        float t0 = 0.f, t1 = 1.f, t2 = 0.f;
        if (BNR) {
            if (in) { t0 = a.bn_coef[c]; t1 = a.bn_coef[2 * a.Cout + c]; t2 = a.bn_coef[3 * a.Cout + c]; }
        } else {
            if (in && a.bias != nullptr) t0 = a.bias[c];
            if (in && a.coef != nullptr) { t1 = a.coef[2 * a.Cout + c]; t2 = a.coef[3 * a.Cout + c]; }
        }
        tab[c] = t0; tab[ctab + c] = t1; tab[2 * ctab + c] = t2;
    }
    int work = pulpo::xcd_remap(blockIdx.x, nwg);
    Tile cur = describe(work);
    int cb = 0;
    float4 wr[2][2];
    {
        const __amdgpu_buffer_rsrc_t rs0 = in_rsrc(cur.b);
        halo_offsets(cur);
#pragma unroll
        for (int tt = 0; tt < 4; ++tt) load_raw(rs0, 0u, tt);
        store_item(smem);
#pragma unroll
        for (int tt = 0; tt < 4; ++tt) load_raw(rs0, kb_bytes, tt);
    }
    __builtin_amdgcn_sched_barrier(0);
#pragma unroll
    for (int pp = 0; pp < 2; ++pp) { wr[pp][0] = load_w(cur.wbase, pp); wr[pp][1] = load_w(cur.wbase, 4 + pp); }
    __syncthreads();

    float4 ra[3], rb[3];

    int pend_tile = -1, pend_co0 = 0;
    auto flush_stats = [&]() {
        stats_store<8, NT>(a.stats != nullptr && pend_tile >= 0, red, a.stats, pend_tile, a.Cout, pend_co0, tid);
        pend_tile = -1;
    };
    for (;;) {
        const int next_work = work + nwg;
        const bool has_next = next_work < nwork;
        const Tile nxt = has_next ? describe(next_work) : cur;

        f32x16 acc[2][4];
#pragma unroll
        for (int p = 0; p < 2; ++p)
#pragma unroll
            for (int x = 0; x < 4; ++x)
#pragma unroll
                for (int r = 0; r < 16; ++r) acc[p][x][r] = 0.f;

        unsigned wcur = cur.wbase;
        for (int chunk = 0; chunk < nchunk; ++chunk) {
            const bool ahead = chunk + 2 >= nchunk;
            const unsigned st_c0 = (unsigned)(ahead ? chunk + 2 - nchunk : chunk + 2) * kb_bytes;
            const __amdgpu_buffer_rsrc_t st_rs = in_rsrc(ahead ? nxt.b : cur.b);
            const float* img_r = smem + cb * Q_IMG;
            float* img_w = smem + (cb ^ 1) * Q_IMG;
            const float* pa = img_r + pa_off;
            const float* pb = img_r + pb_off;
            auto fetch_a = [&](int px) {
                const int o = px * Q_PL * 4;
                ra[0] = *reinterpret_cast<const float4*>(pa + zu + o); rb[0] = *reinterpret_cast<const float4*>(pb + zu + o);
                ra[1] = *reinterpret_cast<const float4*>(pa + zv + o); rb[1] = *reinterpret_cast<const float4*>(pb + zv + o);
                ra[2] = *reinterpret_cast<const float4*>(pa + zw + o); rb[2] = *reinterpret_cast<const float4*>(pb + zw + o);
            };
            const bool last_chunk = chunk + 1 == nchunk;
            const unsigned wnext = last_chunk ? (has_next ? nxt.wbase : cur.wbase) : wcur + w_chunk_stride;
            auto combine = [&](float (&av0)[4], float (&av1)[4]) {
                const f32x2 sav = {sa, sa}, m1 = {-1.f, -1.f}, bwv = {bw, bw};
                f32x2 ylo[3], yhi[3];
#pragma unroll
                for (int p = 0; p < 3; ++p) {
                    ylo[p] = __builtin_elementwise_fma(sav, f32x2{rb[p].x, rb[p].y}, f32x2{ra[p].x, ra[p].y});
                    yhi[p] = __builtin_elementwise_fma(sav, f32x2{rb[p].z, rb[p].w}, f32x2{ra[p].z, ra[p].w});
                }
                const f32x2 lo0 = __builtin_elementwise_fma(m1, ylo[2], ylo[0]), hi0 = __builtin_elementwise_fma(m1, yhi[2], yhi[0]);
                const f32x2 lo1 = __builtin_elementwise_fma(bwv, ylo[2], ylo[1]), hi1 = __builtin_elementwise_fma(bwv, yhi[2], yhi[1]);
                av0[0] = lo0.x; av0[1] = lo0.y; av0[2] = hi0.x; av0[3] = hi0.y;
                av1[0] = lo1.x; av1[1] = lo1.y; av1[2] = hi1.x; av1[3] = hi1.y;
            };
            float avn0[4], avn1[4];
            fetch_a(0);
            combine(avn0, avn1);
            fetch_a(1);
#pragma unroll
            for (int pp = 0; pp < 4; ++pp) {
                const int s0 = pp, s1 = 4 + pp;
                if (((pp + pzh) & 1) != 0) __builtin_amdgcn_s_setprio(1); else __builtin_amdgcn_s_setprio(0);
                const float av0[4] = {avn0[0], avn0[1], avn0[2], avn0[3]}, av1[4] = {avn1[0], avn1[1], avn1[2], avn1[3]};
                const float wv0[4] = {wr[pp & 1][0].x, wr[pp & 1][0].y, wr[pp & 1][0].z, wr[pp & 1][0].w};
                const float wv1[4] = {wr[pp & 1][1].x, wr[pp & 1][1].y, wr[pp & 1][1].z, wr[pp & 1][1].w};
                __builtin_amdgcn_sched_barrier(0);
#pragma unroll
                for (int s2 = 0; s2 < 4; ++s2) {
                    acc[s0 >> 2][s0 & 3] = __builtin_amdgcn_mfma_f32_32x32x2f32(av0[s2], wv0[s2], acc[s0 >> 2][s0 & 3], 0, 0, 0);
                    acc[s1 >> 2][s1 & 3] = __builtin_amdgcn_mfma_f32_32x32x2f32(av1[s2], wv1[s2], acc[s1 >> 2][s1 & 3], 0, 0, 0);
                    if (s2 == 0) {
                        __builtin_amdgcn_sched_barrier(0);
                        if (pp == SP) {
                            store_item(img_w);
                            if (chunk + 2 == nchunk) halo_offsets(has_next ? nxt : cur);
                        }
                        if (pp == SP + 1) { load_raw(st_rs, st_c0, 0); load_raw(st_rs, st_c0, 1); load_raw(st_rs, st_c0, 2); load_raw(st_rs, st_c0, 3); }
                        __builtin_amdgcn_sched_barrier(0);
                    }
                    if (s2 == 1 && pp + 1 < 4) {
                        __builtin_amdgcn_sched_barrier(0);
                        combine(avn0, avn1);
                        __builtin_amdgcn_sched_barrier(0);
                        if (pp + 2 < 4) fetch_a(pp + 2);
                        __builtin_amdgcn_sched_barrier(0);
                    }
                }
                wr[pp & 1][0] = pp < 2 ? load_w(wcur, s0 + 2) : load_w(wnext, s0 - 2);
                wr[pp & 1][1] = pp < 2 ? load_w(wcur, s1 + 2) : load_w(wnext, s1 - 2);
                __builtin_amdgcn_sched_barrier(0);
            }
            wcur += w_chunk_stride;
            __syncthreads();
            cb ^= 1;
            if (chunk == 0) flush_stats();
        }

        float* out_b = a.out + (long)cur.b * a.out_bs;
        const int z0 = cur.z0, y0 = cur.y0, x0 = cur.x0, co0 = cur.co0;
        int elane = lane;
        asm volatile("" : "+v"(elane));
        const int q = elane & 7, kh = (elane >> 3) & 1, g = elane >> 4;
        const float4 zero4 = make_float4(0.f, 0.f, 0.f, 0.f);
        float4 s4 = zero4, q4 = zero4;
        const bool fuse = !BNR && a.coef != nullptr;
        const float4 b4 = BNR ? zero4 : *reinterpret_cast<const float4*>(tab + co0 + 4 * q);
        const float4 bm4 = *reinterpret_cast<const float4*>(tab + co0 + 4 * q);
        const float4 sc4 = *reinterpret_cast<const float4*>(tab + ctab + co0 + 4 * q);
        const float4 sh4 = *reinterpret_cast<const float4*>(tab + 2 * ctab + co0 + 4 * q);
        const float* bn_b = BNR ? a.bn_y + (long)cur.b * a.bn_y_bs + co0 + 4 * q : nullptr;
        const int combo = wave * 4 + g;
        const int ox = combo >> 4, rr = combo & 15;
        const int row = (rr & 3) + 8 * (rr >> 2) + 4 * kh;
        const int vzb = row >> 4, vyb = (row >> 2) & 3, vxb = row & 3;
        float4 yv0 = zero4, yv1 = zero4;
        const bool qok = co0 + 4 * q < a.Cout;
        auto load_y = [&](int oz_) {
            if (BNR && qok) {
                const long vox_ = (long)((z0 + 2 * vzb + oz_) * a.H + y0 + 2 * vyb) * a.W + x0 + 2 * vxb + ox;
                yv0 = *reinterpret_cast<const float4*>(bn_b + vox_ * a.bn_y_ps);
                yv1 = *reinterpret_cast<const float4*>(bn_b + (vox_ + a.W) * a.bn_y_ps);
            }
        };
        load_y(0);
        __builtin_amdgcn_sched_barrier(0);
        f32x2 m1 = {-1.f, -1.f};
        asm volatile("" : "+s"(m1));
#pragma unroll
        for (int p = 0; p < 2; ++p)
#pragma unroll
            for (int r = 0; r < 16; r += 2) {
                const f32x2 a0 = {acc[p][0][r], acc[p][0][r + 1]}, a1 = {acc[p][1][r], acc[p][1][r + 1]};
                const f32x2 a2 = {acc[p][2][r], acc[p][2][r + 1]}, a3 = {acc[p][3][r], acc[p][3][r + 1]};
                const f32x2 o0 = (a0 + a1) + a2, o1 = __builtin_elementwise_fma(m1, a3, __builtin_elementwise_fma(m1, a2, a1));
                acc[p][0][r] = o0.x; acc[p][0][r + 1] = o0.y;
                acc[p][1][r] = o1.x; acc[p][1][r + 1] = o1.y;
            }
#pragma unroll
        for (int oz = 0; oz < 2; ++oz) {
            if (oz > 0) __syncthreads();
            float* const r0 = R + ((wave * 2 + 0) * 16) * 64 + elane;
            float* const r1 = R + ((wave * 2 + 1) * 16) * 64 + elane;
            if (pzh == 0) {
#pragma unroll
                for (int r = 0; r < 16; r += 2) {
                    const f32x2 u0 = f32x2{acc[0][0][r], acc[0][0][r + 1]} + f32x2{acc[1][0][r], acc[1][0][r + 1]};
                    const f32x2 u1 = f32x2{acc[0][1][r], acc[0][1][r + 1]} + f32x2{acc[1][1][r], acc[1][1][r + 1]};
                    r0[r * 64] = oz == 0 ? u0.x : acc[1][0][r]; r0[(r + 1) * 64] = oz == 0 ? u0.y : acc[1][0][r + 1];
                    r1[r * 64] = oz == 0 ? u1.x : acc[1][1][r]; r1[(r + 1) * 64] = oz == 0 ? u1.y : acc[1][1][r + 1];
                }
            } else {
#pragma unroll
                for (int r = 0; r < 16; r += 2) {
                    const f32x2 u0 = __builtin_elementwise_fma(m1, f32x2{acc[0][0][r], acc[0][0][r + 1]}, f32x2{acc[1][0][r], acc[1][0][r + 1]});
                    const f32x2 u1 = __builtin_elementwise_fma(m1, f32x2{acc[0][1][r], acc[0][1][r + 1]}, f32x2{acc[1][1][r], acc[1][1][r + 1]});
                    r0[r * 64] = oz == 0 ? acc[0][0][r] : u0.x; r0[(r + 1) * 64] = oz == 0 ? acc[0][0][r + 1] : u0.y;
                    r1[r * 64] = oz == 0 ? acc[0][1][r] : u1.x; r1[(r + 1) * 64] = oz == 0 ? acc[0][1][r + 1] : u1.y;
                }
            }
            const int gz = z0 + 2 * vzb + oz, gy = y0 + 2 * vyb, gx = x0 + 2 * vxb + ox;
            const long vox = (long)(gz * a.H + gy) * a.W + gx;
            __syncthreads();
            float4 t[4];
#pragma unroll
            for (int p = 0; p < 4; ++p) {
                const float4 u0 = *reinterpret_cast<const float4*>(R + (((0 * 4 + p) * 2 + ox) * 16 + rr) * 64 + kh * 32 + 4 * q);
                const float4 u1 = *reinterpret_cast<const float4*>(R + (((1 * 4 + p) * 2 + ox) * 16 + rr) * 64 + kh * 32 + 4 * q);
                t[p] = make_float4(u0.x + u1.x, u0.y + u1.y, u0.z + u1.z, u0.w + u1.w);
            }
            float4 v0, v1;
            inverse_last(t[0], t[1], t[2], t[3], b4, v0, v1);
            if (BNR) {
                bn_bwd_reduce_pair(v0, v1, yv0, yv1, sc4, sh4, bm4, a.slope, s4, q4);
                if (oz == 0) { __builtin_amdgcn_sched_barrier(0); load_y(1); __builtin_amdgcn_sched_barrier(0); }
            } else {
                stats_add_pair(v0, v1, s4, q4);
            }
            if (fuse) {
                v0 = bn_lrelu4(v0, sc4, sh4, a.slope);
                v1 = bn_lrelu4(v1, sc4, sh4, a.slope);
            }
            float* obase = out_b + (long)((co0 + 4 * q) >> 3) * a.out_kb + ((4 * q) & 7);
            if (qok) {
                *reinterpret_cast<float4*>(obase + vox * a.out_ps) = v0;
                *reinterpret_cast<float4*>(obase + (vox + a.W) * a.out_ps) = v1;
            }
        }
        if (a.stats != nullptr) {
            float* pw_ = part + (wave * 64 + elane) * 8;
            *reinterpret_cast<float4*>(pw_) = s4;
            *reinterpret_cast<float4*>(pw_ + 4) = q4;
            const int c_ = elane & 31, wh_ = elane >> 5;
            const float* pr_ = part + (wave * 64 + (c_ >> 2)) * 8 + wh_ * 4 + (c_ & 3);
            float t_ = 0.f;
#pragma unroll
            for (int j = 0; j < 8; ++j) t_ += pr_[j * 64];
            red[(wave * 2 + wh_) * NT + c_] = t_;
        }
        pend_tile = cur.tile_lin; pend_co0 = co0;
        if (!has_next) break;
        cur = nxt;
        work = next_work;
    }
    __syncthreads();
    flush_stats();
}

template <bool BNR>
__global__ __launch_bounds__(512, 1) void conv3d_k3_wino3_mfma(ConvArgs a) {
    if (__builtin_amdgcn_readfirstlane(threadIdx.x >> 8) != 0) wino3_body<BNR, 2>(a);
    else wino3_body<BNR, 0>(a);
}

__global__ void pack_weight_wino3_kernel(const float* __restrict__ w, float* __restrict__ wp, int Cin, int Cout, int NPad, int dgrad, long total) {
    for (long e = blockIdx.x * (long)blockDim.x + threadIdx.x; e < total; e += (long)gridDim.x * blockDim.x)
        pulpo_conv::pack_wino3_one(w, wp, Cin, Cout, NPad, dgrad, e);
}

constexpr int WINO3_MIN_K = 16;

}

namespace pulpo_conv {

int wino3_shape_ok(int B, int D, int H, int W, int K, int N) {
    const int ncot = (N + Q_NT - 1) / Q_NT;
    if (K < WINO3_MIN_K || K % Q_CH != 0 || N % 4 != 0 || (N % Q_NT != 0 && N < 16) || 3 * ncot * Q_NT > Q_TAB) return 0;
    if (D % 4 != 0 || H % TY != 0 || W % TX != 0) return 0;
    if (conv_tz(D, H, W) != 4) return 0;
    const long items = (long)B * (D / 4) * (H / TY) * (W / TX) * ncot;
    return items >= 256;
}

}

PULPO_API size_t pulpo_conv3d_k3_packed_wino3_floats(int K, int N) { return (size_t)((K + Q_CH - 1) / Q_CH) * 64 * Q_CH * npad(N); }

PULPO_API int pulpo_conv3d_k3_pack_weight_wino3(const float* w, float* wp, int Cin, int Cout, int dgrad, void* stream) {
    PULPO_REQUIRE(w && wp && Cin > 0 && Cout > 0, "conv3d_k3_pack_weight_wino3: bad arguments");
    const int K = dgrad ? Cout : Cin, N = dgrad ? Cin : Cout;
    const long total = (long)((K + Q_CH - 1) / Q_CH) * Q_CH * npad(N);
    const int nb = (int)std::min<long>((total + 255) / 256, 8192);
    hipLaunchKernelGGL(pack_weight_wino3_kernel, dim3(nb), dim3(256), 0, (hipStream_t)stream, w, wp, Cin, Cout, npad(N), dgrad, total);
    return pulpo::check_launch("pack_weight_wino3");
}

static int fwd_wino3_impl(const float* in, int64_t in_bs, int64_t in_ps, int64_t in_cs, const float* wp, const float* bias, const float* coef, float slope,
                          float* out, int64_t out_bs, int64_t out_ps, int64_t out_cs, float* stats, const float* bn_y, int64_t bn_y_bs, int64_t bn_y_ps,
                          const float* bn_coef, int B, int D, int H, int W, int K, int N, void* stream, int64_t in_kb = Q_CH, int64_t out_kb = Q_CH) {
    PULPO_REQUIRE(in && wp && out, "conv3d_k3_fwd_wino3: null pointer");
    PULPO_REQUIRE(B > 0 && K > 0 && N > 0 && D > 0 && D % 4 == 0 && H > 0 && H % TY == 0 && W > 0 && W % TX == 0 && K % Q_CH == 0 && N % 4 == 0 && 3 * ((N + Q_NT - 1) / Q_NT) * Q_NT <= Q_TAB,
                  "conv3d_k3_fwd_wino3: shape %dx%dx%d, %d -> %d channels is not whole 4x8x8 tiles of 8 / 32 channels (see pulpo_conv3d_k3_algo)", D, H, W, K, N);
    PULPO_REQUIRE(K >= 2 * Q_CH, "conv3d_k3_fwd_wino3: at least two 8-channel chunks per tile (%d reduction channels given): the staging runs two chunks ahead", K);
    PULPO_REQUIRE(!stats || conv_tz(D, H, W) == 4, "conv3d_k3_fwd_wino3: %dx%dx%d is tiled 2-deep by pulpo_conv3d_k3_stat_tiles(); this kernel writes 4-deep statistics rows", D, H, W);
    PULPO_REQUIRE(!(coef && stats), "conv3d_k3_fwd_wino3: batch statistics are not available from the fused eval-mode epilogue");
    PULPO_REQUIRE(in_cs == 1 && in_ps % 4 == 0 && in_bs % 4 == 0 && (((uintptr_t)in) & 15) == 0 && (long)D * H * W * in_ps * 4 < (1L << 31) &&
                      in_kb >= Q_CH && in_kb % 4 == 0 && ((long)(K / Q_CH - 1) * in_kb + (long)D * H * W * in_ps) * 4 < (1L << 31),
                  "conv3d_k3_fwd_wino3: the operand must be channels-last (or channel-blocked), 16-byte aligned and smaller than 2 GiB per batch element");
    PULPO_REQUIRE(out_cs == 1 && out_ps % 4 == 0 && out_bs % 4 == 0 && (((uintptr_t)out) & 15) == 0, "conv3d_k3_fwd_wino3: the result must be channels-last, 16-byte aligned");
    PULPO_REQUIRE((((uintptr_t)wp) & 15) == 0, "conv3d_k3_fwd_wino3: packed weights must be 16-byte aligned");
    PULPO_REQUIRE(out_kb >= Q_CH && out_kb % 4 == 0 && (out_kb == Q_CH || N % Q_CH == 0), "conv3d_k3_fwd_wino3: a channel-blocked result needs whole 8-channel blocks");
    ConvArgs a{};
    a.in = in; a.in_bs = in_bs; a.in_ps = in_ps; a.in_cs = in_cs; a.in_kb = in_kb; a.out_kb = out_kb;
    a.wp = wp; a.bias = bias;
    a.out = out; a.out_bs = out_bs; a.out_ps = out_ps; a.out_cs = out_cs;
    a.stats = stats;
    a.coef = coef; a.slope = slope;
    a.bn_y = bn_y; a.bn_y_bs = bn_y_bs; a.bn_y_ps = bn_y_ps; a.bn_coef = bn_coef;
    a.B = B; a.D = D; a.H = H; a.W = W; a.Cin = K; a.Cout = N; a.NPad = npad(N);
    a.ntz = D / 4; a.nty = H / TY; a.ntx = W / TX;
    a.ncot = (N + Q_NT - 1) / Q_NT;
    a.ksplit = 1; a.part = nullptr;
    a.tile_order = (a.ntx % 4 == 0 && a.nty % 4 == 0 && a.ntz % 4 == 0) ? 1 : 0;
    const long nwork = (long)B * a.ntz * a.nty * a.ntx * a.ncot;
    PULPO_REQUIRE(nwork < (1L << 31), "conv3d_k3_fwd_wino3: grid too large");
    hipStream_t st = (hipStream_t)stream;
    const bool bnr = bn_y != nullptr;
    static bool attr_set[2] = {false, false};
    const void* fn = bnr ? reinterpret_cast<const void*>(&conv3d_k3_wino3_mfma<true>) : reinterpret_cast<const void*>(&conv3d_k3_wino3_mfma<false>);
    if (!attr_set[bnr]) {
        hipError_t e = hipFuncSetAttribute(fn, hipFuncAttributeMaxDynamicSharedMemorySize, (int)Q_LDS);
        if (e != hipSuccess) return pulpo::fail((int)e, "hipFuncSetAttribute(conv3d wino3): %s", hipGetErrorString(e));
        attr_set[bnr] = true;
    }
    const int nwg = (int)std::min<long>(nwork, 256);
    if (bnr) hipLaunchKernelGGL((conv3d_k3_wino3_mfma<true>), dim3(nwg), dim3(512), Q_LDS, st, a);
    else hipLaunchKernelGGL((conv3d_k3_wino3_mfma<false>), dim3(nwg), dim3(512), Q_LDS, st, a);
    return pulpo::check_launch("conv3d_k3_wino3_mfma");
}

PULPO_API int pulpo_conv3d_k3_fwd_wino3(const float* in, int64_t in_bs, int64_t in_ps, int64_t in_cs, const float* wp, const float* bias,
                                        const float* coef, float slope, float* out, int64_t out_bs, int64_t out_ps, int64_t out_cs, float* stats, int B,
                                        int D, int H, int W, int K, int N, void* stream) {
    return fwd_wino3_impl(in, in_bs, in_ps, in_cs, wp, bias, coef, slope, out, out_bs, out_ps, out_cs, stats, nullptr, 0, 0, nullptr, B, D, H, W, K, N, stream);
}

PULPO_API int pulpo_conv3d_k3_dgrad_wino3_bnred(const float* in, int64_t in_bs, int64_t in_ps, int64_t in_cs, const float* wp, float* out, int64_t out_bs,
                                                int64_t out_ps, const float* bn_y, int64_t bn_y_bs, int64_t bn_y_ps, const float* bn_coef, float slope,
                                                float* part, int B, int D, int H, int W, int K, int N, void* stream) {
    PULPO_REQUIRE(bn_y && bn_coef && part, "conv3d_k3_dgrad_wino3_bnred: null pointer");
    PULPO_REQUIRE(bn_y_ps % 4 == 0 && bn_y_bs % 4 == 0 && (((uintptr_t)bn_y) & 15) == 0 && (((uintptr_t)bn_coef) & 15) == 0,
                  "conv3d_k3_dgrad_wino3_bnred: pre-norm tensor and coefficients must be channels-last and 16-byte aligned");
    return fwd_wino3_impl(in, in_bs, in_ps, in_cs, wp, nullptr, nullptr, slope, out, out_bs, out_ps, 1, part, bn_y, bn_y_bs, bn_y_ps, bn_coef, B, D, H, W, K, N,
                          stream);
}

PULPO_API int pulpo_conv3d_k3_fwd_wino3_kb(const float* in, int64_t in_bs, int64_t in_ps, int64_t in_kb, const float* wp, const float* bias,
                                           const float* coef, float slope, float* out, int64_t out_bs, int64_t out_ps, int64_t out_kb, float* stats, int B,
                                           int D, int H, int W, int K, int N, void* stream) {
    return fwd_wino3_impl(in, in_bs, in_ps, 1, wp, bias, coef, slope, out, out_bs, out_ps, 1, stats, nullptr, 0, 0, nullptr, B, D, H, W, K, N, stream, in_kb,
                          out_kb);
}

PULPO_API int pulpo_conv3d_k3_dgrad_wino3_bnred_kb(const float* in, int64_t in_bs, int64_t in_ps, int64_t in_kb, const float* wp, float* out, int64_t out_bs,
                                                   int64_t out_ps, int64_t out_kb, const float* bn_y, int64_t bn_y_bs, int64_t bn_y_ps, const float* bn_coef, float slope,
                                                   float* part, int B, int D, int H, int W, int K, int N, void* stream) {
    PULPO_REQUIRE(bn_y && bn_coef && part, "conv3d_k3_dgrad_wino3_bnred_kb: null pointer");
    PULPO_REQUIRE(bn_y_ps % 4 == 0 && bn_y_bs % 4 == 0 && (((uintptr_t)bn_y) & 15) == 0 && (((uintptr_t)bn_coef) & 15) == 0,
                  "conv3d_k3_dgrad_wino3_bnred_kb: pre-norm tensor and coefficients must be channels-last and 16-byte aligned");
    return fwd_wino3_impl(in, in_bs, in_ps, 1, wp, nullptr, nullptr, slope, out, out_bs, out_ps, 1, part, bn_y, bn_y_bs, bn_y_ps, bn_coef, B, D, H, W, K, N,
                          stream, in_kb, out_kb);
}
```

Before: 40.24.

## Add 16-wide MFMA variants for narrow channel tiles in wino3 fwd and wgrad

Adds narrow-channel variants of the Winograd forward/dgrad kernel (when Cout is 16) and of the wgrad w3x kernel (for the last input-channel tile when Cin mod 32 is 16). These use 16x16x4 MFMAs and half-width LDS slots instead of 32x32x2 MFMAs. The goal is to stop wasting half of each 32-wide MFMA tile and half the weight and LDS traffic on zero padding for 16-channel layers. The cost is extra template instantiations, a different LDS layout with padded slot pitches, and more complex epilogue index mapping.

```diff
diff --git a/include/pulpo_hip.h b/include/pulpo_hip.h
--- a/include/pulpo_hip.h
+++ b/include/pulpo_hip.h
@@ -250,6 +250,7 @@
 int pulpo_conv3d_k3_dgrad_wino3_bnred(const float* in, int64_t in_bs, int64_t in_ps, int64_t in_cs, const float* wp, float* out, int64_t out_bs,
                                       int64_t out_ps, const float* bn_y, int64_t bn_y_bs, int64_t bn_y_ps, const float* bn_coef, float slope, float* part,
                                       int B, int D, int H, int W, int K, int N, void* stream);
+int pulpo_conv3d_k3_narrow16(int kind, int K, int N);
 int pulpo_conv3d_k3_wino3g_ok(int B, int D, int H, int W, int K, int N);
 size_t pulpo_conv3d_k3_fwd_wino3g_scratch_floats(int B, int D, int H, int W, int K, int N);
 int pulpo_conv3d_k3_fwd_wino3g(const float* in, int64_t in_bs, int64_t in_ps, int64_t in_cs, const float* wp, const float* bias, const float* coef,
diff --git a/pulpo_amd/csrc/conv3d_wgrad_w2.hip b/pulpo_amd/csrc/conv3d_wgrad_w2.hip
--- a/pulpo_amd/csrc/conv3d_wgrad_w2.hip
+++ b/pulpo_amd/csrc/conv3d_wgrad_w2.hip
@@ -1,10 +1,13 @@
 #include "conv_shared.h"
 #include <type_traits>
 
+PULPO_API int pulpo_conv3d_k3_narrow16(int kind, int K, int N);
+
 namespace {
 
 using namespace pulpo_conv;
 using f32x2 = __attribute__((ext_vector_type(2))) float;
+using f32x4 = __attribute__((ext_vector_type(4))) float;
 
 constexpr int W2G_VROW = 44, W2G_EROW = 36;
 constexpr int W2G_VSLOT = 32 * W2G_VROW, W2G_ESLOT = 32 * W2G_EROW;
@@ -22,6 +25,7 @@
     int nty, ntx, ncit, ncot, nsplit;
     long split_stride;
     long in_kb;
+    int narrow_last;
     long go_kb;
 };
 
@@ -494,14 +498,16 @@
 constexpr size_t W3G_LDS = (size_t)(W2G_VX + W3G_EX) * sizeof(float);
 
 
-template <int SG>
+template <int SG, bool NARROW>
 __device__ __forceinline__ void wgrad_w3x_body(const Wgrad2Args& a) {
     extern __shared__ __attribute__((aligned(16))) float smem[];
+    constexpr int VSL = NARROW ? 16 * W2G_VROW + 2 : W2G_VSLOT, ESL = NARROW ? W2G_ESLOT + 2 : W2G_ESLOT;
+    static_assert(!NARROW || ((VSL * 4) % 512 != 0 && VSL * 4 > 2040 && (ESL * 4) % 512 != 0 && ESL * 4 > 2040 && (16 * VSL + 16 * ESL) * 4 <= (int)W3G_LDS), "slot pitch");
     float* VX = smem;
-    float* EX = smem + W2G_VX;
+    float* EX = smem + (NARROW ? 16 * VSL : W2G_VX);
 
     const int tid = threadIdx.x, lane = tid & 63, wave = __builtin_amdgcn_readfirstlane(tid >> 6);
-    const int i = lane & 31, kk = lane >> 5;
+    const int i = NARROW ? lane & 15 : lane & 31, kk = NARROW ? lane >> 4 : lane >> 5;
     const int py = wave & 3, pxh = wave >> 2;
     const int lid = pulpo::xcd_remap(blockIdx.x, gridDim.x);
     const int npair = a.ncit * a.ncot;
@@ -520,8 +526,8 @@
     const long nstep = (long)ncol * DP;
     const long p_begin = nstep * split / a.nsplit, p_end = nstep * (split + 1) / a.nsplit;
 
-    const bool x_item = tid < 320;
-    const int x_q = tid & 7, x_xb = (tid >> 3) & 3, x_hy = tid >> 5;
+    const bool x_item = NARROW ? tid < 160 : tid < 320;
+    const int x_q = NARROW ? tid & 3 : tid & 7, x_xb = NARROW ? (tid >> 2) & 3 : (tid >> 3) & 3, x_hy = NARROW ? tid >> 4 : tid >> 5;
     const bool e_item = tid >= 256;
     const int e_t = tid - 256;
     const int e_q = e_t & 7, e_xb = (e_t >> 3) & 3, e_y = (e_t >> 5) & 7;
@@ -583,8 +589,9 @@
             const f32x2 sg = px == 1 ? f32x2{1.f, 1.f} : f32x2{-1.f, -1.f};
             const f32x2 lo = f32x2{pa_.x, pa_.y} + sg * f32x2{pb_.x, pb_.y}, hi = f32x2{pa_.z, pa_.w} + sg * f32x2{pb_.z, pb_.w};
             const float4 v = make_float4(lo.x, lo.y, hi.x, hi.y);
-            float* o = x_dst + (px * 4 + slot) * W2G_VSLOT;
-            o[0] = v.x; o[8 * W2G_VROW] = v.y; o[16 * W2G_VROW + x_d4] = v.z; o[24 * W2G_VROW + x_d4] = v.w;
+            float* o = x_dst + (px * 4 + slot) * VSL;
+            if constexpr (NARROW) { o[0] = v.x; o[4 * W2G_VROW] = v.y; o[8 * W2G_VROW] = v.z; o[12 * W2G_VROW] = v.w; }
+            else { o[0] = v.x; o[8 * W2G_VROW] = v.y; o[16 * W2G_VROW + x_d4] = v.z; o[24 * W2G_VROW + x_d4] = v.w; }
         }
     };
     auto write_e = [&](int px, int slot) {
@@ -598,7 +605,7 @@
                 const f32x2 lo = f32x2{d0.x, d0.y} + sg * f32x2{d1.x, d1.y}, hi = f32x2{d0.z, d0.w} + sg * f32x2{d1.z, d1.w};
                 v = make_float4(lo.x, lo.y, hi.x, hi.y);
             }
-            float* o = e_dst + (px * 4 + slot) * W2G_ESLOT;
+            float* o = e_dst + (px * 4 + slot) * ESL;
             o[0] = v.x; o[8 * W2G_EROW] = v.y; o[16 * W2G_EROW + e_d4] = v.z; o[24 * W2G_EROW + e_d4] = v.w;
         }
     };
@@ -609,18 +616,24 @@
         for (int t2 = 0; t2 < 2; ++t2) asm volatile("" : : "v"(er[t2].x), "v"(er[t2].y), "v"(er[t2].z), "v"(er[t2].w));
     };
 
-    f32x16 acc[2][4];
+    constexpr int NH = NARROW ? 2 : 1, NR = NARROW ? 4 : 16;
+    std::conditional_t<NARROW, f32x4, f32x16> acc[2][4][NH];
 #pragma unroll
     for (int p = 0; p < 2; ++p)
 #pragma unroll
         for (int pz = 0; pz < 4; ++pz)
 #pragma unroll
-            for (int r = 0; r < 16; ++r) acc[p][pz][r] = 0.f;
+            for (int nh = 0; nh < NH; ++nh)
+#pragma unroll
+                for (int r = 0; r < NR; ++r) acc[p][pz][nh][r] = 0.f;
 
     const int irow = 8 * (i & 3) + ((i >> 2) ^ (4 * ((i >> 1) & 1)));
-    const float* va = VX + irow * W2G_VROW + (2 * kk + ta) * 4;
-    const float* vb = VX + irow * W2G_VROW + (2 * kk + tb) * 4;
-    const float* ea = EX + irow * W2G_EROW + (2 * kk) * 4;
+    const int krow = NARROW ? 2 * (kk >> 1) : 2 * kk, kcol = NARROW ? 2 * (kk & 1) : 0;
+    const int vrow = NARROW ? 4 * (i & 3) + (i >> 2) : irow;
+    const float* va = VX + vrow * W2G_VROW + (krow + ta) * 4 + kcol;
+    const float* vb = VX + vrow * W2G_VROW + (krow + tb) * 4 + kcol;
+    const float* ea = EX + irow * W2G_EROW + krow * 4 + kcol;
+    const int e_hi = ((irow ^ 4) - irow) * W2G_EROW;
 
     long p = p_begin;
     while (p < p_end) {
@@ -653,15 +666,31 @@
 #pragma unroll
             for (int gi = 0; gi < 4; ++gi) {
                 const int g = gi >> 1, px = 2 * pxh + (gi & 1), pl = gi & 1;
-                const float* eb0 = ea + (px * 4 + d0s) * W2G_ESLOT + g * 16;
-                const float* eb1 = ea + (px * 4 + d1s) * W2G_ESLOT + g * 16;
-                e0[0] = *reinterpret_cast<const float4*>(eb0 + 4 * ea_); e1[0] = *reinterpret_cast<const float4*>(eb0 + 4 * eb_);
-                e0[1] = *reinterpret_cast<const float4*>(eb1 + 4 * ea_); e1[1] = *reinterpret_cast<const float4*>(eb1 + 4 * eb_);
-#pragma unroll
-                for (int dz = 0; dz < 3; ++dz) {
-                    const int off = (px * 4 + ((HM + dz) & 3)) * W2G_VSLOT + g * 16;
-                    av[dz] = *reinterpret_cast<const float4*>(va + off);
-                    bv[dz] = *reinterpret_cast<const float4*>(vb + off);
+                const float* eb0 = ea + (px * 4 + d0s) * ESL + g * 16;
+                const float* eb1 = ea + (px * 4 + d1s) * ESL + g * 16;
+                if constexpr (NARROW) {
+                    auto two = [&](const float* p_) {
+                        const float2 lo = *reinterpret_cast<const float2*>(p_), hi = *reinterpret_cast<const float2*>(p_ + e_hi);
+                        return make_float4(lo.x, lo.y, hi.x, hi.y);
+                    };
+                    e0[0] = two(eb0 + 4 * ea_); e1[0] = two(eb0 + 4 * eb_);
+                    e0[1] = two(eb1 + 4 * ea_); e1[1] = two(eb1 + 4 * eb_);
+#pragma unroll
+                    for (int dz = 0; dz < 3; ++dz) {
+                        const int off = (px * 4 + ((HM + dz) & 3)) * VSL + g * 16;
+                        const float2 a2 = *reinterpret_cast<const float2*>(va + off), b2 = *reinterpret_cast<const float2*>(vb + off);
+                        av[dz] = make_float4(a2.x, a2.y, 0.f, 0.f);
+                        bv[dz] = make_float4(b2.x, b2.y, 0.f, 0.f);
+                    }
+                } else {
+                    e0[0] = *reinterpret_cast<const float4*>(eb0 + 4 * ea_); e1[0] = *reinterpret_cast<const float4*>(eb0 + 4 * eb_);
+                    e0[1] = *reinterpret_cast<const float4*>(eb1 + 4 * ea_); e1[1] = *reinterpret_cast<const float4*>(eb1 + 4 * eb_);
+#pragma unroll
+                    for (int dz = 0; dz < 3; ++dz) {
+                        const int off = (px * 4 + ((HM + dz) & 3)) * VSL + g * 16;
+                        av[dz] = *reinterpret_cast<const float4*>(va + off);
+                        bv[dz] = *reinterpret_cast<const float4*>(vb + off);
+                    }
                 }
                 __builtin_amdgcn_sched_barrier(0);
                 const f32x2 sev = {se, se}, sav = {sa, sa};
@@ -689,8 +718,14 @@
                 constexpr int PZA = HB ? 2 : 0, PZB = HB ? 3 : 1;
 #pragma unroll
                 for (int s_ = 0; s_ < 4; ++s_) {
-                    acc[pl][PZA] = __builtin_amdgcn_mfma_f32_32x32x2f32(va4[s_], ea4[s_], acc[pl][PZA], 0, 0, 0);
-                    acc[pl][PZB] = __builtin_amdgcn_mfma_f32_32x32x2f32(vb4[s_], eb4[s_], acc[pl][PZB], 0, 0, 0);
+                    if constexpr (NARROW) {
+                        const int nh = s_ & 1, ks = s_ >> 1;
+                        acc[pl][PZA][nh] = __builtin_amdgcn_mfma_f32_16x16x4f32(va4[ks], ea4[2 * nh + ks], acc[pl][PZA][nh], 0, 0, 0);
+                        acc[pl][PZB][nh] = __builtin_amdgcn_mfma_f32_16x16x4f32(vb4[ks], eb4[2 * nh + ks], acc[pl][PZB][nh], 0, 0, 0);
+                    } else {
+                        acc[pl][PZA][0] = __builtin_amdgcn_mfma_f32_32x32x2f32(va4[s_], ea4[s_], acc[pl][PZA][0], 0, 0, 0);
+                        acc[pl][PZB][0] = __builtin_amdgcn_mfma_f32_32x32x2f32(vb4[s_], eb4[s_], acc[pl][PZB][0], 0, 0, 0);
+                    }
                     if (s_ == 0 && gi >= SG && gi < SG + 2) {
                         __builtin_amdgcn_sched_barrier(0);
                         if (gi == SG) touch_raw();
@@ -727,28 +762,31 @@
     __syncthreads();
     float* X = smem;
     const int Cc = min(32, a.Cin - ci0);
+    constexpr int XR = NH * NR;
 #pragma unroll 1
     for (int dz = 0; dz < 3; ++dz) {
 #pragma unroll
-        for (int r = 0; r < 16; ++r) {
-            const float h0 = 0.5f * (acc[0][1][r] + acc[0][2][r]), h1 = 0.5f * (acc[1][1][r] + acc[1][2][r]);
-            const float m0 = dz == 0 ? acc[0][0][r] + h0 : dz == 1 ? 0.5f * (acc[0][1][r] - acc[0][2][r]) : h0 + acc[0][3][r];
-            const float m1 = dz == 0 ? acc[1][0][r] + h1 : dz == 1 ? 0.5f * (acc[1][1][r] - acc[1][2][r]) : h1 + acc[1][3][r];
+        for (int rr = 0; rr < XR; ++rr) {
+            const int nh = rr / NR, r = rr % NR;
+            const float h0 = 0.5f * (acc[0][1][nh][r] + acc[0][2][nh][r]), h1 = 0.5f * (acc[1][1][nh][r] + acc[1][2][nh][r]);
+            const float m0 = dz == 0 ? acc[0][0][nh][r] + h0 : dz == 1 ? 0.5f * (acc[0][1][nh][r] - acc[0][2][nh][r]) : h0 + acc[0][3][nh][r];
+            const float m1 = dz == 0 ? acc[1][0][nh][r] + h1 : dz == 1 ? 0.5f * (acc[1][1][nh][r] - acc[1][2][nh][r]) : h1 + acc[1][3][nh][r];
             float t0, t1, t2;
             if (pxh == 0) { t0 = m0 + 0.5f * m1; t1 = 0.5f * m1; t2 = 0.5f * m1; }
             else { t0 = 0.5f * m0; t1 = -0.5f * m0; t2 = 0.5f * m0 + m1; }
-            X[((wave * 3 + 0) * 16 + r) * 64 + lane] = t0;
-            X[((wave * 3 + 1) * 16 + r) * 64 + lane] = t1;
-            X[((wave * 3 + 2) * 16 + r) * 64 + lane] = t2;
+            X[((wave * 3 + 0) * XR + rr) * 64 + lane] = t0;
+            X[((wave * 3 + 1) * XR + rr) * 64 + lane] = t1;
+            X[((wave * 3 + 2) * XR + rr) * 64 + lane] = t2;
         }
         __syncthreads();
-        for (int e = tid; e < 3 * 16 * 64; e += 512) {
-            const int l = e & 63, r = (e >> 6) & 15, kx = e >> 10;
+        for (int e = tid; e < 3 * XR * 64; e += 512) {
+            const int l = e & 63, r = (e >> 6) % XR, kx = e / (64 * XR);
             float s[4];
 #pragma unroll
             for (int q = 0; q < 4; ++q)
-                s[q] = X[((q * 3 + kx) * 16 + r) * 64 + l] + X[(((q + 4) * 3 + kx) * 16 + r) * 64 + l];
-            const int ci = (r & 3) + 8 * (r >> 2) + 4 * (l >> 5), co = co0 + (l & 31);
+                s[q] = X[((q * 3 + kx) * XR + r) * 64 + l] + X[(((q + 4) * 3 + kx) * XR + r) * 64 + l];
+            const int ci = NARROW ? 4 * (l >> 4) + (r & 3) : (r & 3) + 8 * (r >> 2) + 4 * (l >> 5);
+            const int co = NARROW ? co0 + 16 * (r >> 2) + (l & 15) : co0 + (l & 31);
             if (ci < Cc && co < a.Cout) {
                 const float hs = 0.5f * (s[1] + s[2]);
                 float* d = a.dwp + (long)split * a.split_stride + ((long)((dz * 3 + 0) * 3 + kx) * a.Cin + ci0 + ci) * a.NPad + co;
@@ -764,8 +802,15 @@
 
 template <int DUMMY>
 __global__ __launch_bounds__(512, 2) void conv3d_k3_wgrad_w3x(Wgrad2Args a) {
-    if (__builtin_amdgcn_readfirstlane(threadIdx.x >> 8) != 0) wgrad_w3x_body<2>(a);
-    else wgrad_w3x_body<0>(a);
+    const int pair = pulpo::xcd_remap(blockIdx.x, gridDim.x) % (a.ncit * a.ncot);
+    const bool narrow = a.narrow_last != 0 && pair / a.ncot == a.ncit - 1;
+    if (__builtin_amdgcn_readfirstlane(threadIdx.x >> 8) != 0) {
+        if (narrow) wgrad_w3x_body<2, true>(a);
+        else wgrad_w3x_body<2, false>(a);
+    } else {
+        if (narrow) wgrad_w3x_body<0, true>(a);
+        else wgrad_w3x_body<0, false>(a);
+    }
 }
 
 }
@@ -802,6 +847,7 @@
     a.B = B; a.D = D; a.H = H; a.W = W; a.Cin = Cin; a.Cout = Cout; a.NPad = npad(Cout);
     a.nty = pulpo::cdiv(H, 8); a.ntx = pulpo::cdiv(W, 8);
     a.ncit = pulpo::cdiv(Cin, 32); a.ncot = pulpo::cdiv(Cout, 32);
+    a.narrow_last = pulpo_conv3d_k3_narrow16(1, Cin, Cout);
     const int npair = a.ncit * a.ncot;
     const long nstep = (long)B * a.nty * a.ntx * D;
     int nsplit = wgrad_w2_splits(npair, nstep, max_workgroups);
diff --git a/pulpo_amd/csrc/conv3d_wino3.hip b/pulpo_amd/csrc/conv3d_wino3.hip
--- a/pulpo_amd/csrc/conv3d_wino3.hip
+++ b/pulpo_amd/csrc/conv3d_wino3.hip
@@ -6,6 +6,7 @@
 
 using namespace pulpo_conv;
 using f32x2 = __attribute__((ext_vector_type(2))) float;
+using f32x4 = __attribute__((ext_vector_type(4))) float;
 
 constexpr int Q_CH = 8, Q_NT = 32;
 constexpr int Q_PL = HY * 4;
@@ -22,7 +23,10 @@
 static_assert(Q_LDS <= 160 * 1024, "one workgroup per CU");
 
 
-template <bool BNR, int SP>
+__device__ __forceinline__ void unpack_w(const float4& w, float (&v)[4]) { v[0] = w.x; v[1] = w.y; v[2] = w.z; v[3] = w.w; }
+__device__ __forceinline__ void unpack_w(const float2& w, float (&v)[4]) { v[0] = w.x; v[1] = w.y; v[2] = 0.f; v[3] = 0.f; }
+
+template <bool BNR, int SP, bool N16>
 __device__ __forceinline__ void wino3_body(const ConvArgs& a) {
     constexpr int CH = Q_CH, NT = Q_NT;
     extern __shared__ __attribute__((aligned(16))) float smem[];
@@ -32,8 +36,8 @@
     float* const part = red + Q_RED;
 
     const int tid = threadIdx.x, lane = tid & 63, wave = __builtin_amdgcn_readfirstlane(tid >> 6);
-    const int i = lane & 31, kk = lane >> 5;
-    const int py = wave & 3, pzh = wave >> 2;
+    const int i = N16 ? lane & 15 : lane & 31, kk = N16 ? lane >> 4 : lane >> 5;
+    const int py = wave & 3, pzh = N16 ? SP / 2 : wave >> 2;
     const int nchunk = a.Cin / CH;
     const int nwork = a.B * a.ntz * a.nty * a.ntx * a.ncot;
     const int nwg = gridDim.x;
@@ -57,9 +61,10 @@
     const float sa = tab_s(py);
     const int zu = (pzh == 0 ? 0 : 2) * Q_PLROWS * 4, zv = (pzh == 0 ? 1 : 3) * Q_PLROWS * 4, zw = (pzh == 0 ? 2 : 1) * Q_PLROWS * 4;
     const float bw = pzh == 0 ? 1.f : -1.f;
-    const int lrow = (i >> 4) * 2 * Q_PLROWS + ((i >> 2) & 3) * 8 + (i & 3);
-    const int pa_off = (kk * Q_QROWS + lrow + ta * 4) * 4;
-    const int pb_off = (kk * Q_QROWS + lrow + tb * 4) * 4;
+    const int lrow = N16 ? (i >> 3) * 2 * Q_PLROWS + ((i >> 2) & 1) * 8 + (i & 3) : (i >> 4) * 2 * Q_PLROWS + ((i >> 2) & 3) * 8 + (i & 3);
+    const int pa_off = N16 ? ((kk >> 1) * Q_QROWS + lrow + ta * 4) * 4 + 2 * (kk & 1) : (kk * Q_QROWS + lrow + ta * 4) * 4;
+    const int pb_off = N16 ? ((kk >> 1) * Q_QROWS + lrow + tb * 4) * 4 + 2 * (kk & 1) : (kk * Q_QROWS + lrow + tb * 4) * 4;
+    constexpr int A_HALF = 2 * 8 * 4;
 
     constexpr unsigned OOB = 0x80000000u;
     const __amdgpu_buffer_rsrc_t w_rsrc = __builtin_amdgcn_make_buffer_rsrc(const_cast<float*>(a.wp), 0, -1, 0x00020000);
@@ -123,9 +128,12 @@
     };
     const unsigned w_chunk_stride = 64u * CH * a.NPad * 4u;
     const unsigned w_pt_stride = (unsigned)CH * a.NPad * 4u;
-    const int wl_off = (i * CH + 4 * kk) * 4;
+    const int wl_off = N16 ? (i * CH + 2 * kk) * 4 : (i * CH + 4 * kk) * 4;
+    using wrow_t = std::conditional_t<N16, float2, float4>;
     auto load_w = [&](unsigned wofs, int s) {
-        return __builtin_bit_cast(float4, __builtin_amdgcn_raw_buffer_load_b128(w_rsrc, wl_off, (int)(wofs + ((s >> 2) * 16 + (s & 3)) * w_pt_stride), 0));
+        const int so = (int)(wofs + ((s >> 2) * 16 + (s & 3)) * w_pt_stride);
+        if constexpr (N16) return __builtin_bit_cast(float2, __builtin_amdgcn_raw_buffer_load_b64(w_rsrc, wl_off, so, 0));
+        else return __builtin_bit_cast(float4, __builtin_amdgcn_raw_buffer_load_b128(w_rsrc, wl_off, so, 0));
     };
 
     const int ctab = a.ncot * NT;
@@ -143,7 +151,8 @@
     int work = pulpo::xcd_remap(blockIdx.x, nwg);
     Tile cur = describe(work);
     int cb = 0;
-    float4 wr[2][2];
+    constexpr int WRING = N16 ? 4 : 2;
+    wrow_t wr[WRING][2];
     {
         const __amdgpu_buffer_rsrc_t rs0 = in_rsrc(cur.b);
         halo_offsets(cur);
@@ -155,7 +164,7 @@
     }
     __builtin_amdgcn_sched_barrier(0);
 #pragma unroll
-    for (int pp = 0; pp < 2; ++pp) { wr[pp][0] = load_w(cur.wbase, pp); wr[pp][1] = load_w(cur.wbase, 4 + pp); }
+    for (int pp = 0; pp < WRING; ++pp) { wr[pp][0] = load_w(cur.wbase, pp); wr[pp][1] = load_w(cur.wbase, 4 + pp); }
     __syncthreads();
 
     float4 ra[3], rb[3];
@@ -170,13 +179,16 @@
         const bool has_next = next_work < nwork;
         const Tile nxt = has_next ? describe(next_work) : cur;
 
-        f32x16 acc[2][4];
+        constexpr int NH = N16 ? 2 : 1, NR = N16 ? 4 : 16;
+        std::conditional_t<N16, f32x4, f32x16> acc[2][4][NH];
 #pragma unroll
         for (int p = 0; p < 2; ++p)
 #pragma unroll
             for (int x = 0; x < 4; ++x)
 #pragma unroll
-                for (int r = 0; r < 16; ++r) acc[p][x][r] = 0.f;
+                for (int h = 0; h < NH; ++h)
+#pragma unroll
+                    for (int r = 0; r < NR; ++r) acc[p][x][h][r] = 0.f;
 
         unsigned wcur = cur.wbase;
         for (int chunk = 0; chunk < nchunk; ++chunk) {
@@ -187,8 +199,22 @@
             float* img_w = smem + (cb ^ 1) * Q_IMG;
             const float* pa = img_r + pa_off;
             const float* pb = img_r + pb_off;
+            int a_half = A_HALF;
+            if constexpr (N16) asm volatile("" : "+v"(a_half));
+            const float* pa_h = pa + a_half;
+            const float* pb_h = pb + a_half;
             auto fetch_a = [&](int px) {
                 const int o = px * Q_PL * 4;
+                if constexpr (N16) {
+                    auto two = [](const float* p_, const float* h_) {
+                        const float2 lo = *reinterpret_cast<const float2*>(p_), hi = *reinterpret_cast<const float2*>(h_);
+                        return make_float4(lo.x, lo.y, hi.x, hi.y);
+                    };
+                    ra[0] = two(pa + zu + o, pa_h + zu + o); rb[0] = two(pb + zu + o, pb_h + zu + o);
+                    ra[1] = two(pa + zv + o, pa_h + zv + o); rb[1] = two(pb + zv + o, pb_h + zv + o);
+                    ra[2] = two(pa + zw + o, pa_h + zw + o); rb[2] = two(pb + zw + o, pb_h + zw + o);
+                    return;
+                }
                 ra[0] = *reinterpret_cast<const float4*>(pa + zu + o); rb[0] = *reinterpret_cast<const float4*>(pb + zu + o);
                 ra[1] = *reinterpret_cast<const float4*>(pa + zv + o); rb[1] = *reinterpret_cast<const float4*>(pb + zv + o);
                 ra[2] = *reinterpret_cast<const float4*>(pa + zw + o); rb[2] = *reinterpret_cast<const float4*>(pb + zw + o);
@@ -211,26 +237,34 @@
             float avn0[4], avn1[4];
             fetch_a(0);
             combine(avn0, avn1);
+            if constexpr (N16) __builtin_amdgcn_sched_barrier(0);
             fetch_a(1);
 #pragma unroll
             for (int pp = 0; pp < 4; ++pp) {
                 const int s0 = pp, s1 = 4 + pp;
                 if (((pp + pzh) & 1) != 0) __builtin_amdgcn_s_setprio(1); else __builtin_amdgcn_s_setprio(0);
                 const float av0[4] = {avn0[0], avn0[1], avn0[2], avn0[3]}, av1[4] = {avn1[0], avn1[1], avn1[2], avn1[3]};
-                const float wv0[4] = {wr[pp & 1][0].x, wr[pp & 1][0].y, wr[pp & 1][0].z, wr[pp & 1][0].w};
-                const float wv1[4] = {wr[pp & 1][1].x, wr[pp & 1][1].y, wr[pp & 1][1].z, wr[pp & 1][1].w};
+                float wv0[4], wv1[4];
+                unpack_w(wr[pp % WRING][0], wv0);
+                unpack_w(wr[pp % WRING][1], wv1);
                 __builtin_amdgcn_sched_barrier(0);
 #pragma unroll
                 for (int s2 = 0; s2 < 4; ++s2) {
-                    acc[s0 >> 2][s0 & 3] = __builtin_amdgcn_mfma_f32_32x32x2f32(av0[s2], wv0[s2], acc[s0 >> 2][s0 & 3], 0, 0, 0);
-                    acc[s1 >> 2][s1 & 3] = __builtin_amdgcn_mfma_f32_32x32x2f32(av1[s2], wv1[s2], acc[s1 >> 2][s1 & 3], 0, 0, 0);
+                    if constexpr (N16) {
+                        const int hf = s2 & 1, ks = s2 >> 1;
+                        acc[0][pp][hf] = __builtin_amdgcn_mfma_f32_16x16x4f32(av0[2 * hf + ks], wv0[ks], acc[0][pp][hf], 0, 0, 0);
+                        acc[1][pp][hf] = __builtin_amdgcn_mfma_f32_16x16x4f32(av1[2 * hf + ks], wv1[ks], acc[1][pp][hf], 0, 0, 0);
+                    } else {
+                        acc[s0 >> 2][s0 & 3][0] = __builtin_amdgcn_mfma_f32_32x32x2f32(av0[s2], wv0[s2], acc[s0 >> 2][s0 & 3][0], 0, 0, 0);
+                        acc[s1 >> 2][s1 & 3][0] = __builtin_amdgcn_mfma_f32_32x32x2f32(av1[s2], wv1[s2], acc[s1 >> 2][s1 & 3][0], 0, 0, 0);
+                    }
                     if (s2 == 0) {
                         __builtin_amdgcn_sched_barrier(0);
                         if (pp == SP) {
                             store_item(img_w);
                             if (chunk + 2 == nchunk) halo_offsets(has_next ? nxt : cur);
                         }
-                        if (pp == SP + 1) { load_raw(st_rs, st_c0, 0); load_raw(st_rs, st_c0, 1); load_raw(st_rs, st_c0, 2); load_raw(st_rs, st_c0, 3); }
+                        if (pp == (N16 ? SP : SP + 1)) { load_raw(st_rs, st_c0, 0); load_raw(st_rs, st_c0, 1); load_raw(st_rs, st_c0, 2); load_raw(st_rs, st_c0, 3); }
                         __builtin_amdgcn_sched_barrier(0);
                     }
                     if (s2 == 1 && pp + 1 < 4) {
@@ -241,8 +275,13 @@
                         __builtin_amdgcn_sched_barrier(0);
                     }
                 }
-                wr[pp & 1][0] = pp < 2 ? load_w(wcur, s0 + 2) : load_w(wnext, s0 - 2);
-                wr[pp & 1][1] = pp < 2 ? load_w(wcur, s1 + 2) : load_w(wnext, s1 - 2);
+                if constexpr (N16) {
+                    wr[pp][0] = load_w(wnext, s0);
+                    wr[pp][1] = load_w(wnext, s1);
+                } else {
+                    wr[pp & 1][0] = pp < 2 ? load_w(wcur, s0 + 2) : load_w(wnext, s0 - 2);
+                    wr[pp & 1][1] = pp < 2 ? load_w(wcur, s1 + 2) : load_w(wnext, s1 - 2);
+                }
                 __builtin_amdgcn_sched_barrier(0);
             }
             wcur += w_chunk_stride;
@@ -255,82 +294,65 @@
         const int z0 = cur.z0, y0 = cur.y0, x0 = cur.x0, co0 = cur.co0;
         int elane = lane;
         asm volatile("" : "+v"(elane));
-        const int q = elane & 7, kh = (elane >> 3) & 1, g = elane >> 4;
         const float4 zero4 = make_float4(0.f, 0.f, 0.f, 0.f);
         float4 s4 = zero4, q4 = zero4;
         const bool fuse = !BNR && a.coef != nullptr;
-        const float4 b4 = BNR ? zero4 : *reinterpret_cast<const float4*>(tab + co0 + 4 * q);
-        const float4 bm4 = *reinterpret_cast<const float4*>(tab + co0 + 4 * q);
-        const float4 sc4 = *reinterpret_cast<const float4*>(tab + ctab + co0 + 4 * q);
-        const float4 sh4 = *reinterpret_cast<const float4*>(tab + 2 * ctab + co0 + 4 * q);
-        const float* bn_b = BNR ? a.bn_y + (long)cur.b * a.bn_y_bs + co0 + 4 * q : nullptr;
-        const int combo = wave * 4 + g;
-        const int ox = combo >> 4, rr = combo & 15;
-        const int row = (rr & 3) + 8 * (rr >> 2) + 4 * kh;
-        const int vzb = row >> 4, vyb = (row >> 2) & 3, vxb = row & 3;
-        float4 yv0 = zero4, yv1 = zero4;
-        const bool qok = co0 + 4 * q < a.Cout;
-        auto load_y = [&](int oz_) {
-            if (BNR && qok) {
-                const long vox_ = (long)((z0 + 2 * vzb + oz_) * a.H + y0 + 2 * vyb) * a.W + x0 + 2 * vxb + ox;
-                yv0 = *reinterpret_cast<const float4*>(bn_b + vox_ * a.bn_y_ps);
-                yv1 = *reinterpret_cast<const float4*>(bn_b + (vox_ + a.W) * a.bn_y_ps);
-            }
-        };
-        load_y(0);
-        __builtin_amdgcn_sched_barrier(0);
-        f32x2 m1 = {-1.f, -1.f};
-        asm volatile("" : "+s"(m1));
-#pragma unroll
-        for (int p = 0; p < 2; ++p)
-#pragma unroll
-            for (int r = 0; r < 16; r += 2) {
-                const f32x2 a0 = {acc[p][0][r], acc[p][0][r + 1]}, a1 = {acc[p][1][r], acc[p][1][r + 1]};
-                const f32x2 a2 = {acc[p][2][r], acc[p][2][r + 1]}, a3 = {acc[p][3][r], acc[p][3][r + 1]};
-                const f32x2 o0 = (a0 + a1) + a2, o1 = __builtin_elementwise_fma(m1, a3, __builtin_elementwise_fma(m1, a2, a1));
-                acc[p][0][r] = o0.x; acc[p][0][r + 1] = o0.y;
-                acc[p][1][r] = o1.x; acc[p][1][r + 1] = o1.y;
-            }
-#pragma unroll
-        for (int oz = 0; oz < 2; ++oz) {
-            if (oz > 0) __syncthreads();
-            float* const r0 = R + ((wave * 2 + 0) * 16) * 64 + elane;
-            float* const r1 = R + ((wave * 2 + 1) * 16) * 64 + elane;
-            if (pzh == 0) {
-#pragma unroll
-                for (int r = 0; r < 16; r += 2) {
-                    const f32x2 u0 = f32x2{acc[0][0][r], acc[0][0][r + 1]} + f32x2{acc[1][0][r], acc[1][0][r + 1]};
-                    const f32x2 u1 = f32x2{acc[0][1][r], acc[0][1][r + 1]} + f32x2{acc[1][1][r], acc[1][1][r + 1]};
-                    r0[r * 64] = oz == 0 ? u0.x : acc[1][0][r]; r0[(r + 1) * 64] = oz == 0 ? u0.y : acc[1][0][r + 1];
-                    r1[r * 64] = oz == 0 ? u1.x : acc[1][1][r]; r1[(r + 1) * 64] = oz == 0 ? u1.y : acc[1][1][r + 1];
-                }
-            } else {
-#pragma unroll
-                for (int r = 0; r < 16; r += 2) {
-                    const f32x2 u0 = __builtin_elementwise_fma(m1, f32x2{acc[0][0][r], acc[0][0][r + 1]}, f32x2{acc[1][0][r], acc[1][0][r + 1]});
-                    const f32x2 u1 = __builtin_elementwise_fma(m1, f32x2{acc[0][1][r], acc[0][1][r + 1]}, f32x2{acc[1][1][r], acc[1][1][r + 1]});
-                    r0[r * 64] = oz == 0 ? acc[0][0][r] : u0.x; r0[(r + 1) * 64] = oz == 0 ? acc[0][0][r + 1] : u0.y;
-                    r1[r * 64] = oz == 0 ? acc[0][1][r] : u1.x; r1[(r + 1) * 64] = oz == 0 ? acc[0][1][r + 1] : u1.y;
-                }
-            }
+        if constexpr (N16) {
+            const int q = elane & 3, vzb = (elane >> 3) & 1, vxb = elane >> 4;
+            const int hf_ = wave & 1, ox = (wave >> 1) & 1, oz = wave >> 2;
+            const int vyb = 2 * hf_ + ((elane >> 2) & 1);
+            const float4 b4 = BNR ? zero4 : *reinterpret_cast<const float4*>(tab + co0 + 4 * q);
+            const float4 bm4 = *reinterpret_cast<const float4*>(tab + co0 + 4 * q);
+            const float4 sc4 = *reinterpret_cast<const float4*>(tab + ctab + co0 + 4 * q);
+            const float4 sh4 = *reinterpret_cast<const float4*>(tab + 2 * ctab + co0 + 4 * q);
+            const bool qok = co0 + 4 * q < a.Cout;
             const int gz = z0 + 2 * vzb + oz, gy = y0 + 2 * vyb, gx = x0 + 2 * vxb + ox;
             const long vox = (long)(gz * a.H + gy) * a.W + gx;
+            float4 yv0 = zero4, yv1 = zero4;
+            if (BNR && qok) {
+                const float* bn_b = a.bn_y + (long)cur.b * a.bn_y_bs + co0 + 4 * q;
+                yv0 = *reinterpret_cast<const float4*>(bn_b + vox * a.bn_y_ps);
+                yv1 = *reinterpret_cast<const float4*>(bn_b + (vox + a.W) * a.bn_y_ps);
+            }
+            __builtin_amdgcn_sched_barrier(0);
+            f32x2 m1 = {-1.f, -1.f};
+            asm volatile("" : "+s"(m1));
+#pragma unroll
+            for (int p = 0; p < 2; ++p)
+#pragma unroll
+                for (int hf = 0; hf < 2; ++hf)
+#pragma unroll
+                    for (int r = 0; r < 4; r += 2) {
+                        const f32x2 a0 = {acc[p][0][hf][r], acc[p][0][hf][r + 1]}, a1 = {acc[p][1][hf][r], acc[p][1][hf][r + 1]};
+                        const f32x2 a2 = {acc[p][2][hf][r], acc[p][2][hf][r + 1]}, a3 = {acc[p][3][hf][r], acc[p][3][hf][r + 1]};
+                        const f32x2 o0 = (a0 + a1) + a2, o1 = __builtin_elementwise_fma(m1, a3, __builtin_elementwise_fma(m1, a2, a1));
+                        acc[p][0][hf][r] = o0.x; acc[p][0][hf][r + 1] = o0.y;
+                        acc[p][1][hf][r] = o1.x; acc[p][1][hf][r + 1] = o1.y;
+                    }
+#pragma unroll
+            for (int x = 0; x < 2; ++x)
+#pragma unroll
+                for (int hf = 0; hf < 2; ++hf)
+#pragma unroll
+                    for (int r = 0; r < 4; ++r) {
+                        const float c0 = acc[0][x][hf][r], c1 = acc[1][x][hf][r];
+                        float* const w0 = R + (((0 * 8 + wave) * 2 + x) * 8 + hf * 4 + r) * 64 + elane;
+                        float* const w1 = R + (((1 * 8 + wave) * 2 + x) * 8 + hf * 4 + r) * 64 + elane;
+                        if (pzh == 0) { *w0 = c0 + c1; *w1 = c1; }
+                        else { *w0 = c0; *w1 = c1 - c0; }
+                    }
             __syncthreads();
             float4 t[4];
 #pragma unroll
             for (int p = 0; p < 4; ++p) {
-                const float4 u0 = *reinterpret_cast<const float4*>(R + (((0 * 4 + p) * 2 + ox) * 16 + rr) * 64 + kh * 32 + 4 * q);
-                const float4 u1 = *reinterpret_cast<const float4*>(R + (((1 * 4 + p) * 2 + ox) * 16 + rr) * 64 + kh * 32 + 4 * q);
+                const float4 u0 = *reinterpret_cast<const float4*>(R + (((oz * 8 + p) * 2 + ox) * 8 + hf_ * 4 + vxb) * 64 + 4 * (elane & 15));
+                const float4 u1 = *reinterpret_cast<const float4*>(R + (((oz * 8 + 4 + p) * 2 + ox) * 8 + hf_ * 4 + vxb) * 64 + 4 * (elane & 15));
                 t[p] = make_float4(u0.x + u1.x, u0.y + u1.y, u0.z + u1.z, u0.w + u1.w);
             }
             float4 v0, v1;
             inverse_last(t[0], t[1], t[2], t[3], b4, v0, v1);
-            if (BNR) {
-                bn_bwd_reduce_pair(v0, v1, yv0, yv1, sc4, sh4, bm4, a.slope, s4, q4);
-                if (oz == 0) { __builtin_amdgcn_sched_barrier(0); load_y(1); __builtin_amdgcn_sched_barrier(0); }
-            } else {
-                stats_add_pair(v0, v1, s4, q4);
-            }
+            if (BNR) bn_bwd_reduce_pair(v0, v1, yv0, yv1, sc4, sh4, bm4, a.slope, s4, q4);
+            else stats_add_pair(v0, v1, s4, q4);
             if (fuse) {
                 v0 = bn_lrelu4(v0, sc4, sh4, a.slope);
                 v1 = bn_lrelu4(v1, sc4, sh4, a.slope);
@@ -340,17 +362,112 @@
                 *reinterpret_cast<float4*>(obase + vox * a.out_ps) = v0;
                 *reinterpret_cast<float4*>(obase + (vox + a.W) * a.out_ps) = v1;
             }
-        }
-        if (a.stats != nullptr) {
-            float* pw_ = part + (wave * 64 + elane) * 8;
-            *reinterpret_cast<float4*>(pw_) = s4;
-            *reinterpret_cast<float4*>(pw_ + 4) = q4;
-            const int c_ = elane & 31, wh_ = elane >> 5;
-            const float* pr_ = part + (wave * 64 + (c_ >> 2)) * 8 + wh_ * 4 + (c_ & 3);
-            float t_ = 0.f;
-#pragma unroll
-            for (int j = 0; j < 8; ++j) t_ += pr_[j * 64];
-            red[(wave * 2 + wh_) * NT + c_] = t_;
+            if (a.stats != nullptr) {
+                float* pw_ = part + (wave * 64 + elane) * 8;
+                *reinterpret_cast<float4*>(pw_) = s4;
+                *reinterpret_cast<float4*>(pw_ + 4) = q4;
+                const int c_ = elane & 31, wh_ = elane >> 5;
+                const float* pr_ = part + (wave * 64 + ((c_ >> 2) & 3)) * 8 + wh_ * 4 + (c_ & 3);
+                float t_ = 0.f;
+#pragma unroll
+                for (int j = 0; j < 16; ++j) t_ += pr_[j * 32];
+                red[(wave * 2 + wh_) * NT + c_] = c_ < 16 ? t_ : 0.f;
+            }
+        } else {
+            const int q = elane & 7, kh = (elane >> 3) & 1, g = elane >> 4;
+            const float4 b4 = BNR ? zero4 : *reinterpret_cast<const float4*>(tab + co0 + 4 * q);
+            const float4 bm4 = *reinterpret_cast<const float4*>(tab + co0 + 4 * q);
+            const float4 sc4 = *reinterpret_cast<const float4*>(tab + ctab + co0 + 4 * q);
+            const float4 sh4 = *reinterpret_cast<const float4*>(tab + 2 * ctab + co0 + 4 * q);
+            const float* bn_b = BNR ? a.bn_y + (long)cur.b * a.bn_y_bs + co0 + 4 * q : nullptr;
+            const int combo = wave * 4 + g;
+            const int ox = combo >> 4, rr = combo & 15;
+            const int row = (rr & 3) + 8 * (rr >> 2) + 4 * kh;
+            const int vzb = row >> 4, vyb = (row >> 2) & 3, vxb = row & 3;
+            float4 yv0 = zero4, yv1 = zero4;
+            const bool qok = co0 + 4 * q < a.Cout;
+            auto load_y = [&](int oz_) {
+                if (BNR && qok) {
+                    const long vox_ = (long)((z0 + 2 * vzb + oz_) * a.H + y0 + 2 * vyb) * a.W + x0 + 2 * vxb + ox;
+                    yv0 = *reinterpret_cast<const float4*>(bn_b + vox_ * a.bn_y_ps);
+                    yv1 = *reinterpret_cast<const float4*>(bn_b + (vox_ + a.W) * a.bn_y_ps);
+                }
+            };
+            load_y(0);
+            __builtin_amdgcn_sched_barrier(0);
+            f32x2 m1 = {-1.f, -1.f};
+            asm volatile("" : "+s"(m1));
+#pragma unroll
+            for (int p = 0; p < 2; ++p)
+#pragma unroll
+                for (int r = 0; r < 16; r += 2) {
+                    const f32x2 a0 = {acc[p][0][0][r], acc[p][0][0][r + 1]}, a1 = {acc[p][1][0][r], acc[p][1][0][r + 1]};
+                    const f32x2 a2 = {acc[p][2][0][r], acc[p][2][0][r + 1]}, a3 = {acc[p][3][0][r], acc[p][3][0][r + 1]};
+                    const f32x2 o0 = (a0 + a1) + a2, o1 = __builtin_elementwise_fma(m1, a3, __builtin_elementwise_fma(m1, a2, a1));
+                    acc[p][0][0][r] = o0.x; acc[p][0][0][r + 1] = o0.y;
+                    acc[p][1][0][r] = o1.x; acc[p][1][0][r + 1] = o1.y;
+                }
+#pragma unroll
+            for (int oz = 0; oz < 2; ++oz) {
+                if (oz > 0) __syncthreads();
+                float* const r0 = R + ((wave * 2 + 0) * 16) * 64 + elane;
+                float* const r1 = R + ((wave * 2 + 1) * 16) * 64 + elane;
+                if (pzh == 0) {
+#pragma unroll
+                    for (int r = 0; r < 16; r += 2) {
+                        const f32x2 u0 = f32x2{acc[0][0][0][r], acc[0][0][0][r + 1]} + f32x2{acc[1][0][0][r], acc[1][0][0][r + 1]};
+                        const f32x2 u1 = f32x2{acc[0][1][0][r], acc[0][1][0][r + 1]} + f32x2{acc[1][1][0][r], acc[1][1][0][r + 1]};
+                        r0[r * 64] = oz == 0 ? u0.x : acc[1][0][0][r]; r0[(r + 1) * 64] = oz == 0 ? u0.y : acc[1][0][0][r + 1];
+                        r1[r * 64] = oz == 0 ? u1.x : acc[1][1][0][r]; r1[(r + 1) * 64] = oz == 0 ? u1.y : acc[1][1][0][r + 1];
+                    }
+                } else {
+#pragma unroll
+                    for (int r = 0; r < 16; r += 2) {
+                        const f32x2 u0 = __builtin_elementwise_fma(m1, f32x2{acc[0][0][0][r], acc[0][0][0][r + 1]}, f32x2{acc[1][0][0][r], acc[1][0][0][r + 1]});
+                        const f32x2 u1 = __builtin_elementwise_fma(m1, f32x2{acc[0][1][0][r], acc[0][1][0][r + 1]}, f32x2{acc[1][1][0][r], acc[1][1][0][r + 1]});
+                        r0[r * 64] = oz == 0 ? acc[0][0][0][r] : u0.x; r0[(r + 1) * 64] = oz == 0 ? acc[0][0][0][r + 1] : u0.y;
+                        r1[r * 64] = oz == 0 ? acc[0][1][0][r] : u1.x; r1[(r + 1) * 64] = oz == 0 ? acc[0][1][0][r + 1] : u1.y;
+                    }
+                }
+                const int gz = z0 + 2 * vzb + oz, gy = y0 + 2 * vyb, gx = x0 + 2 * vxb + ox;
+                const long vox = (long)(gz * a.H + gy) * a.W + gx;
+                __syncthreads();
+                float4 t[4];
+#pragma unroll
+                for (int p = 0; p < 4; ++p) {
+                    const float4 u0 = *reinterpret_cast<const float4*>(R + (((0 * 4 + p) * 2 + ox) * 16 + rr) * 64 + kh * 32 + 4 * q);
+                    const float4 u1 = *reinterpret_cast<const float4*>(R + (((1 * 4 + p) * 2 + ox) * 16 + rr) * 64 + kh * 32 + 4 * q);
+                    t[p] = make_float4(u0.x + u1.x, u0.y + u1.y, u0.z + u1.z, u0.w + u1.w);
+                }
+                float4 v0, v1;
+                inverse_last(t[0], t[1], t[2], t[3], b4, v0, v1);
+                if (BNR) {
+                    bn_bwd_reduce_pair(v0, v1, yv0, yv1, sc4, sh4, bm4, a.slope, s4, q4);
+                    if (oz == 0) { __builtin_amdgcn_sched_barrier(0); load_y(1); __builtin_amdgcn_sched_barrier(0); }
+                } else {
+                    stats_add_pair(v0, v1, s4, q4);
+                }
+                if (fuse) {
+                    v0 = bn_lrelu4(v0, sc4, sh4, a.slope);
+                    v1 = bn_lrelu4(v1, sc4, sh4, a.slope);
+                }
+                float* obase = out_b + (long)((co0 + 4 * q) >> 3) * a.out_kb + ((4 * q) & 7);
+                if (qok) {
+                    *reinterpret_cast<float4*>(obase + vox * a.out_ps) = v0;
+                    *reinterpret_cast<float4*>(obase + (vox + a.W) * a.out_ps) = v1;
+                }
+            }
+            if (a.stats != nullptr) {
+                float* pw_ = part + (wave * 64 + elane) * 8;
+                *reinterpret_cast<float4*>(pw_) = s4;
+                *reinterpret_cast<float4*>(pw_ + 4) = q4;
+                const int c_ = elane & 31, wh_ = elane >> 5;
+                const float* pr_ = part + (wave * 64 + (c_ >> 2)) * 8 + wh_ * 4 + (c_ & 3);
+                float t_ = 0.f;
+#pragma unroll
+                for (int j = 0; j < 8; ++j) t_ += pr_[j * 64];
+                red[(wave * 2 + wh_) * NT + c_] = t_;
+            }
         }
         pend_tile = cur.tile_lin; pend_co0 = co0;
         if (!has_next) break;
@@ -361,10 +478,10 @@
     flush_stats();
 }
 
-template <bool BNR>
+template <bool BNR, bool N16>
 __global__ __launch_bounds__(512, 1) void conv3d_k3_wino3_mfma(ConvArgs a) {
-    if (__builtin_amdgcn_readfirstlane(threadIdx.x >> 8) != 0) wino3_body<BNR, 2>(a);
-    else wino3_body<BNR, 0>(a);
+    if (__builtin_amdgcn_readfirstlane(threadIdx.x >> 8) != 0) wino3_body<BNR, 2, N16>(a);
+    else wino3_body<BNR, 0, N16>(a);
 }
 
 __global__ void pack_weight_wino3_kernel(const float* __restrict__ w, float* __restrict__ wp, int Cin, int Cout, int NPad, int dgrad, long total) {
@@ -387,6 +504,12 @@
     return items >= 256;
 }
 
+}
+
+PULPO_API int pulpo_conv3d_k3_narrow16(int kind, int K, int N) {
+    if (kind == 0) return K >= WINO3_MIN_K && K % Q_CH == 0 && N == 16;
+    if (kind == 1) return K > 0 && N > 0 && K % 32 == 16;
+    return 0;
 }
 
 PULPO_API size_t pulpo_conv3d_k3_packed_wino3_floats(int K, int N) { return (size_t)((K + Q_CH - 1) / Q_CH) * 64 * Q_CH * npad(N); }
@@ -431,16 +554,19 @@
     PULPO_REQUIRE(nwork < (1L << 31), "conv3d_k3_fwd_wino3: grid too large");
     hipStream_t st = (hipStream_t)stream;
     const bool bnr = bn_y != nullptr;
-    static bool attr_set[2] = {false, false};
-    const void* fn = bnr ? reinterpret_cast<const void*>(&conv3d_k3_wino3_mfma<true>) : reinterpret_cast<const void*>(&conv3d_k3_wino3_mfma<false>);
-    if (!attr_set[bnr]) {
-        hipError_t e = hipFuncSetAttribute(fn, hipFuncAttributeMaxDynamicSharedMemorySize, (int)Q_LDS);
+    const bool n16 = pulpo_conv3d_k3_narrow16(0, K, N) != 0;
+    using kernel_t = void (*)(ConvArgs);
+    static const kernel_t kernels[2][2] = {{conv3d_k3_wino3_mfma<false, false>, conv3d_k3_wino3_mfma<false, true>},
+                                           {conv3d_k3_wino3_mfma<true, false>, conv3d_k3_wino3_mfma<true, true>}};
+    static bool attr_set[2][2] = {{false, false}, {false, false}};
+    const kernel_t fn = kernels[bnr][n16];
+    if (!attr_set[bnr][n16]) {
+        hipError_t e = hipFuncSetAttribute(reinterpret_cast<const void*>(fn), hipFuncAttributeMaxDynamicSharedMemorySize, (int)Q_LDS);
         if (e != hipSuccess) return pulpo::fail((int)e, "hipFuncSetAttribute(conv3d wino3): %s", hipGetErrorString(e));
-        attr_set[bnr] = true;
+        attr_set[bnr][n16] = true;
     }
     const int nwg = (int)std::min<long>(nwork, 256);
-    if (bnr) hipLaunchKernelGGL((conv3d_k3_wino3_mfma<true>), dim3(nwg), dim3(512), Q_LDS, st, a);
-    else hipLaunchKernelGGL((conv3d_k3_wino3_mfma<false>), dim3(nwg), dim3(512), Q_LDS, st, a);
+    hipLaunchKernelGGL(fn, dim3(nwg), dim3(512), Q_LDS, st, a);
     return pulpo::check_launch("conv3d_k3_wino3_mfma");
 }
 
```

Result: faster. 40.65 (median of 6 runs) (+1.0%).
